# yoraish/mmd

Hardware: AMD Instinct MI355X
Metric: guided trajectories/sec (H=64, 100 denoise steps), 32-robot Empty map (higher is better)
Workload: dtype f32 (f16x2 split on the fp16 MFMA pipe: every fp32 product as 3 fp16 MFMAs, fp32 accumulate)

## Files before the change

include/mmd_amd_debug.h:

```cpp
#ifndef MMD_AMD_DEBUG_H
#define MMD_AMD_DEBUG_H

#include <stddef.h>
#include <stdint.h>

#include "mmd_amd.h"

#ifdef __cplusplus
extern "C" {
#endif

typedef struct mmd_profiler_s* mmd_profiler_t;
int mmd_profiler_create(mmd_profiler_t* out, int max_launches, int stride);
int mmd_profiler_destroy(mmd_profiler_t p);
int mmd_profiler_create_windowed(mmd_profiler_t* out, int max_launches, int stride, int window, int period);
enum { MMD_PROF_UNET = 0, MMD_PROF_STEP_GUIDED = 1, MMD_PROF_STEP_PLAIN = 2, MMD_PROF_UNET_FUSED = 3 };
int mmd_profiler_intervals(mmd_profiler_t p, int kind, double* start_ms, double* end_ms, int cap, int* n_out);
int mmd_profiler_read(mmd_profiler_t p, double* mean_ms, int* n_launches);

double mmd_unet_flops_per_trajectory(void);
double mmd_unet_mfma_flops_per_trajectory(void);
double mmd_unet_f16x2_flops_per_trajectory(void);

int mmd_sampler_stream_chunks(int n_streams, int n_robots, int samples_per_robot);

int mmd_unet_forward_profiled(mmd_unet_t unet, const float* x_dev, int t, float* eps_dev, int n_traj,
                              void* workspace_dev, size_t workspace_bytes, mmd_profiler_t profiler, void* stream);

size_t mmd_unet_weight_bytes(mmd_unet_t unet);

int mmd_unet_precision(mmd_unet_t unet);

#define MMD_TRACE_WORDS 12
int mmd_debug_ddpm_step_trace(mmd_unet_t unet, const mmd_sampler_desc* s, const mmd_guide_desc* guide, float* x_dev,
                              const float* hard_dev, int n_robots, int samples_per_robot, int i, const float* noise_dev,
                              uint64_t seed, uint32_t draw_index, void* workspace_dev, size_t workspace_bytes,
                              float* mu_dev, float* guide_chain_dev, uint32_t* trace_dev, void* stream);

#ifdef __cplusplus
}
#endif
#endif
```

mmd_amd/_lib.py:

```python
import ctypes as C
import os

_HERE = os.path.dirname(os.path.abspath(__file__))
LIB_PATH = os.path.join(_HERE, "lib", "libmmd_amd.so")
ABI_VERSION = 9
HARD_ROWS_START_GOAL = (1 << 63) | 1


def signed64(mask):
    mask = int(mask) & 0xFFFFFFFFFFFFFFFF
    return mask - (1 << 64) if mask >> 63 else mask



class ConsBins(C.Structure):
    _fields_ = [
        ("lo", C.c_float * 2), ("inv_cell", C.c_float * 2),
        ("nx", C.c_int32), ("ny", C.c_int32), ("n_all", C.c_int32), ("robot0", C.c_int32),
        ("radius", C.c_float), ("weight", C.c_float),
        ("cell_off_dev", C.c_void_p), ("entries_dev", C.c_void_p),
    ]


class GuideDesc(C.Structure):
    _fields_ = [
        ("norm_min", C.c_float * 4), ("norm_max", C.c_float * 4),
        ("limits_lo", C.c_float * 2), ("limits_hi", C.c_float * 2),
        ("grid_nx", C.c_int32), ("grid_ny", C.c_int32), ("n_grids", C.c_int32), ("n_maps", C.c_int32),
        ("sdf_grids_dev", C.c_void_p), ("robot_map_dev", C.c_void_p),
        ("ws_min", C.c_float * 2), ("ws_max", C.c_float * 2),
        ("margin", C.c_float), ("dt", C.c_float), ("sigma_gp", C.c_float),
        ("weight_collision", C.c_float), ("weight_smoothness", C.c_float), ("max_grad_norm", C.c_float),
        ("cons_ell_dev", C.c_void_p), ("grp_slot_off_dev", C.c_void_p), ("grp_weight_dev", C.c_void_p),
        ("robot_grp_off_dev", C.c_void_p), ("max_slots_per_robot", C.c_int32), ("cons_uniform_radius", C.c_float),
        ("extra_spheres_dev", C.c_void_p), ("extra_boxes_dev", C.c_void_p),
        ("n_extra_spheres", C.c_int32), ("n_extra_boxes", C.c_int32),
        ("clip_grad_rule", C.c_int32), ("max_grad_value", C.c_float),
        ("cons_bins", C.POINTER(ConsBins)),
    ]


class SamplerDesc(C.Structure):
    _fields_ = [
        ("n_diffusion_steps", C.c_int32),
        ("sqrt_recip_alphas_cumprod", C.POINTER(C.c_float)),
        ("sqrt_recipm1_alphas_cumprod", C.POINTER(C.c_float)),
        ("posterior_mean_coef1", C.POINTER(C.c_float)),
        ("posterior_mean_coef2", C.POINTER(C.c_float)),
        ("posterior_log_variance_clipped", C.POINTER(C.c_float)),
        ("n_guide_steps", C.c_int32), ("t_start_guide", C.c_int32),
        ("noise_std_extra", C.c_float), ("hard_rows", C.c_uint64), ("n_streams", C.c_int32),
        ("traj_index_base", C.c_int64), ("noise_std_extra_by_t", C.POINTER(C.c_float)), ("profiler", C.c_void_p),
        ("scale_grad_by_std", C.c_int32), ("model_predicts_x0", C.c_int32),
        ("flags", C.c_uint32), ("guide_coop_max", C.c_int32), ("robot_seeds_dev", C.c_void_p),
    ]


SAMPLER_NO_FUSED_STEP, SAMPLER_PERSIST = 1, 2
UNET_LAYERED, UNET_LAYERED_VALU = 1, 2
UNET_PRECISION_F32, UNET_PRECISION_F16 = 0, 1
UNET_PRECISIONS = {"f32": UNET_PRECISION_F32, "f16": UNET_PRECISION_F16}


class UnetOptions(C.Structure):
    _fields_ = [("flags", C.c_uint32), ("rtb_fused", C.c_int32), ("mconv_max_cs", C.c_int32), ("two_per_workgroup_max", C.c_int32),
                ("precision", C.c_int32)]


class EnsembleTile(C.Structure):
    _fields_ = [
        ("unet", C.c_void_p), ("sampler", C.POINTER(SamplerDesc)), ("guide", C.POINTER(GuideDesc)),
        ("x_dev", C.c_void_p), ("hard_dev", C.c_void_p), ("step_noise_dev", C.c_void_p), ("chain_dev", C.c_void_p),
        ("seed", C.c_uint64),
    ]


class CrossCond(C.Structure):
    _fields_ = [("m1", C.c_int32), ("m2", C.c_int32), ("ind1", C.c_int32), ("ind2", C.c_int32),
                ("rel", C.c_float * 4), ("boundary", C.c_float * 4), ("by_robot_dev", C.c_void_p)]


class AgentPath(C.Structure):
    _fields_ = [("batch_dev", C.c_void_p), ("index", C.c_int32), ("length", C.c_int32), ("start_time", C.c_int32),
                ("reserved", C.c_int32)]


class Conflict(C.Structure):
    _fields_ = [("t", C.c_int32), ("a", C.c_int32), ("b", C.c_int32), ("reserved", C.c_int32), ("pa", C.c_float * 2),
                ("pb", C.c_float * 2), ("mid", C.c_float * 2), ("reserved2", C.c_float * 2)]


class TileRef(C.Structure):
    _fields_ = [("agent", C.c_int32), ("t0", C.c_int32), ("offset", C.c_float * 2), ("rule", C.c_int32), ("reserved", C.c_int32)]


ADHERENCE_LINE, ADHERENCE_HIGHWAYS, ADHERENCE_CONVEYOR, ADHERENCE_DROP_REGION = 0, 1, 2, 3
CONFLICTS_ORDERED, CONFLICTS_PAIRS = 0, 1
SELECT_CBS, SELECT_PP = 0, 1
REPLAN_CONFLICTED, REPLAN_INDEPENDENT = 0, 1


_SIGNATURES = {
    "mmd_abi_version": (C.c_int, []),
    "mmd_last_error": (C.c_char_p, []),
    "mmd_unet_num_tensors": (C.c_int, [C.c_int, C.c_int]),
    "mmd_unet_tensor_numel": (C.c_int64, [C.c_int, C.c_int, C.c_int]),
    "mmd_unet_create": (C.c_int, [C.POINTER(C.c_void_p), C.c_int, C.c_int, C.c_int, C.POINTER(C.c_void_p),
                                  C.POINTER(C.c_int64), C.c_int, C.POINTER(UnetOptions), C.c_void_p]),
    "mmd_unet_destroy": (C.c_int, [C.c_void_p]),
    "mmd_unet_workspace_bytes": (C.c_size_t, [C.c_void_p, C.c_int]),
    "mmd_unet_forward": (C.c_int, [C.c_void_p, C.c_void_p, C.c_int, C.c_void_p, C.c_int, C.c_void_p, C.c_size_t,
                                   C.c_void_p]),
    "mmd_pack_constraints": (C.c_int, [C.c_int, C.POINTER(C.c_int32), C.POINTER(C.c_void_p), C.POINTER(C.c_void_p),
                                       C.POINTER(C.c_void_p), C.c_int, C.c_void_p, C.c_int, C.POINTER(C.c_int32)]),
    "mmd_soft_constraints_from_paths": (C.c_int, [C.c_void_p, C.c_int, C.c_int, C.c_int, C.c_int, C.c_float, C.c_float,
                                                  C.c_void_p, C.c_void_p, C.c_void_p, C.c_void_p, C.c_void_p]),
    "mmd_cons_bins_bytes": (C.c_size_t, [C.c_int, C.c_int, C.c_int, C.POINTER(C.c_size_t), C.POINTER(C.c_size_t)]),
    "mmd_bin_constraints_from_paths": (C.c_int, [C.c_void_p, C.c_int, C.c_int, C.c_float, C.POINTER(C.c_float), C.POINTER(C.c_float),
                                                 C.c_int, C.c_int, C.c_void_p, C.c_void_p, C.c_void_p]),
    "mmd_bin_paths": (C.c_int, [C.c_void_p, C.c_int, C.c_int, C.c_float, C.POINTER(C.c_float), C.POINTER(C.c_float), C.c_int, C.c_int,
                                C.c_int, C.c_void_p, C.c_void_p, C.c_void_p]),
    "mmd_guide_steps": (C.c_int, [C.POINTER(GuideDesc), C.c_void_p, C.c_void_p, C.c_uint64, C.c_int, C.c_int, C.c_int,
                                  C.c_void_p, C.c_void_p]),
    "mmd_sampler_workspace_bytes": (C.c_size_t, [C.c_void_p, C.c_int]),
    "mmd_ddpm_step": (C.c_int, [C.c_void_p, C.POINTER(SamplerDesc), C.POINTER(GuideDesc), C.c_void_p, C.c_void_p,
                                C.c_int, C.c_int, C.c_int, C.c_void_p, C.c_uint64, C.c_uint32, C.c_void_p, C.c_size_t,
                                C.c_void_p]),
    "mmd_p_sample_loop": (C.c_int, [C.c_void_p, C.POINTER(SamplerDesc), C.POINTER(GuideDesc), C.c_void_p, C.c_void_p,
                                    C.c_int, C.c_int, C.c_int, C.c_int, C.c_int, C.c_void_p, C.c_uint64, C.c_void_p,
                                    C.c_void_p, C.c_size_t, C.c_void_p]),
    "mmd_ddim_sample": (C.c_int, [C.c_void_p, C.POINTER(SamplerDesc), C.c_void_p, C.c_void_p, C.c_int, C.POINTER(GuideDesc),
                                  C.c_void_p, C.c_void_p, C.c_int, C.c_int, C.c_int, C.c_uint64, C.c_void_p, C.c_void_p,
                                  C.c_size_t, C.c_void_p]),
    "mmd_p_sample_loop_ensemble": (C.c_int, [C.POINTER(EnsembleTile), C.c_int, C.POINTER(CrossCond), C.c_int, C.c_int,
                                             C.c_int, C.c_int, C.c_int, C.c_int, C.c_void_p, C.c_size_t, C.c_void_p]),
    "mmd_q_sample": (C.c_int, [C.c_void_p, C.c_void_p, C.c_void_p, C.c_float, C.c_float, C.c_uint64, C.c_uint32,
                               C.c_int64, C.c_int, C.c_void_p]),
    "mmd_rr_collisions": (C.c_int, [C.c_void_p, C.c_int, C.c_int, C.c_float, C.c_void_p, C.c_void_p, C.c_void_p]),
    "mmd_count_collisions": (C.c_int, [C.c_void_p, C.c_void_p, C.c_int, C.c_int, C.c_int, C.c_int, C.c_int, C.c_float,
                                       C.c_void_p, C.c_void_p]),
    "mmd_count_collisions_binned": (C.c_int, [C.c_void_p, C.POINTER(ConsBins), C.c_int, C.c_int, C.c_float, C.c_void_p, C.c_void_p]),
    "mmd_path_conflicts_binned": (C.c_int, [C.c_void_p, C.POINTER(ConsBins), C.c_int, C.c_float, C.c_void_p, C.c_void_p, C.c_void_p,
                                            C.c_void_p, C.c_void_p, C.c_int, C.c_void_p]),
    "mmd_find_conflicts": (C.c_int, [C.c_void_p, C.c_int, C.c_int, C.c_float, C.c_int, C.c_void_p, C.c_void_p, C.c_void_p,
                                     C.c_void_p, C.c_int, C.c_void_p]),
    "mmd_scan_candidates": (C.c_int, [C.c_void_p, C.c_int, C.c_int, C.c_int, C.c_void_p, C.c_void_p, C.c_int, C.c_float, C.c_int,
                                      C.c_int, C.c_void_p, C.c_void_p, C.c_void_p, C.c_void_p]),
    "mmd_path_constraints": (C.c_int, [C.c_void_p, C.c_int, C.c_int, C.c_int, C.c_int, C.c_int, C.c_int, C.c_float, C.c_float,
                                       C.c_int, C.c_void_p, C.c_void_p, C.c_void_p, C.c_void_p, C.c_void_p]),
    "mmd_round_constraints_init": (C.c_int, [C.c_int, C.c_int, C.c_int, C.c_int, C.c_float, C.c_float, C.c_void_p, C.c_void_p, C.c_void_p,
                                             C.c_void_p, C.c_void_p, C.c_void_p, C.c_void_p]),
    "mmd_round_soft_from_paths": (C.c_int, [C.c_void_p, C.c_int, C.c_int, C.c_int, C.c_int, C.c_int, C.c_float, C.c_void_p, C.c_void_p]),
    "mmd_conflict_constraints_append": (C.c_int, [C.c_void_p, C.POINTER(ConsBins), C.c_int, C.c_int, C.c_int, C.c_int, C.c_float, C.c_float,
                                                  C.c_void_p, C.c_void_p, C.c_void_p, C.c_void_p]),
    "mmd_round_select": (C.c_int, [C.c_void_p, C.POINTER(ConsBins), C.c_void_p, C.c_int, C.c_int, C.c_float, C.c_int, C.c_int, C.c_void_p,
                                   C.c_void_p, C.c_void_p, C.c_void_p, C.c_void_p]),
    "mmd_framed_constraints_from_paths": (C.c_int, [C.c_void_p, C.c_void_p, C.c_int, C.c_int, C.c_int, C.c_int, C.c_int, C.c_float, C.c_float,
                                                    C.POINTER(C.c_float), C.POINTER(C.c_float), C.c_void_p, C.c_void_p, C.c_void_p, C.c_void_p,
                                                    C.c_void_p, C.c_void_p, C.c_void_p]),
    "mmd_solution_stats": (C.c_int, [C.c_void_p, C.c_int, C.c_int, C.c_float, C.c_void_p, C.c_int, C.c_void_p, C.c_void_p, C.c_void_p]),
    "mmd_postprocess_trajs": (C.c_int, [C.POINTER(GuideDesc), C.c_void_p, C.c_int, C.c_int, C.c_int, C.c_int,
                                        C.POINTER(C.c_float), C.c_float, C.POINTER(C.c_float), C.POINTER(C.c_float), C.c_int,
                                        C.c_void_p, C.c_int, C.c_void_p, C.c_void_p, C.c_void_p, C.c_void_p, C.c_void_p,
                                        C.c_void_p]),
    "mmd_select_best": (C.c_int, [C.c_void_p, C.c_void_p, C.c_void_p, C.c_void_p, C.c_int, C.c_int, C.c_void_p, C.c_void_p,
                                  C.c_void_p, C.c_void_p]),
    "mmd_points_collision": (C.c_int, [C.POINTER(GuideDesc), C.c_void_p, C.c_int, C.c_int, C.c_int, C.c_float, C.c_void_p,
                                       C.c_void_p]),
    "mmd_variance_waypoints": (C.c_int, [C.c_void_p, C.c_int, C.c_int, C.c_void_p, C.c_void_p]),
    "mmd_unnormalize_trajs": (C.c_int, [C.c_void_p, C.c_size_t, C.c_size_t, C.c_size_t, C.POINTER(C.c_float), C.POINTER(C.c_float),
                                        C.c_float, C.c_void_p, C.c_void_p, C.c_void_p]),
    "mmd_cross_condition": (C.c_int, [C.c_void_p, C.c_void_p, C.c_int, C.c_int, C.POINTER(C.c_float),
                                      C.POINTER(C.c_float), C.c_int, C.c_void_p]),
}

_DEBUG_SIGNATURES = {
    "mmd_profiler_create": (C.c_int, [C.POINTER(C.c_void_p), C.c_int, C.c_int]),
    "mmd_profiler_create_windowed": (C.c_int, [C.POINTER(C.c_void_p), C.c_int, C.c_int, C.c_int, C.c_int]),
    "mmd_profiler_intervals": (C.c_int, [C.c_void_p, C.c_int, C.POINTER(C.c_double), C.POINTER(C.c_double), C.c_int,
                                         C.POINTER(C.c_int)]),
    "mmd_profiler_destroy": (C.c_int, [C.c_void_p]),
    "mmd_profiler_read": (C.c_int, [C.c_void_p, C.POINTER(C.c_double), C.POINTER(C.c_int)]),
    "mmd_sampler_stream_chunks": (C.c_int, [C.c_int, C.c_int, C.c_int]),
    "mmd_unet_flops_per_trajectory": (C.c_double, []),
    "mmd_unet_mfma_flops_per_trajectory": (C.c_double, []),
    "mmd_unet_f16x2_flops_per_trajectory": (C.c_double, []),
    "mmd_unet_forward_profiled": (C.c_int, [C.c_void_p, C.c_void_p, C.c_int, C.c_void_p, C.c_int, C.c_void_p, C.c_size_t,
                                            C.c_void_p, C.c_void_p]),
    "mmd_unet_weight_bytes": (C.c_size_t, [C.c_void_p]),
    "mmd_unet_precision": (C.c_int, [C.c_void_p]),
    "mmd_debug_ddpm_step_trace": (C.c_int, [C.c_void_p, C.POINTER(SamplerDesc), C.POINTER(GuideDesc), C.c_void_p, C.c_void_p,
                                            C.c_int, C.c_int, C.c_int, C.c_void_p, C.c_uint64, C.c_uint32, C.c_void_p, C.c_size_t,
                                            C.c_void_p, C.c_void_p, C.c_void_p, C.c_void_p]),
}
TRACE_WORDS = 12

EXPORTED_SYMBOLS = tuple(_SIGNATURES)
DEBUG_SYMBOLS = tuple(_DEBUG_SIGNATURES)
_lib = None


def load():
    global _lib
    if _lib is None:
        if not os.path.exists(LIB_PATH):
            raise ImportError(f"{LIB_PATH} not found: the HIP extension is required (run ./build.sh or "
                              f"`python -c 'import __graft_entry__ as g; g.build()'`); there is no CPU fallback")
        lib = C.CDLL(LIB_PATH)
        for name, (res, args) in list(_SIGNATURES.items()) + list(_DEBUG_SIGNATURES.items()):
            fn = getattr(lib, name)
            fn.restype, fn.argtypes = res, args
        if lib.mmd_abi_version() != ABI_VERSION:
            raise ImportError(f"libmmd_amd.so ABI {lib.mmd_abi_version()} != expected {ABI_VERSION}")
        _lib = lib
    return _lib


def check(rc):
    if rc != 0:
        raise RuntimeError("libmmd_amd: " + load().mmd_last_error().decode())


def raw_stream(device_index=None):
    import torch
    if device_index is None:
        device_index = torch.cuda.current_device()
    get = getattr(torch._C, "_cuda_getCurrentRawStream", None)
    return int(get(device_index)) if get is not None else int(torch.cuda.current_stream(device_index).cuda_stream)


def current_stream_ptr():
    return C.c_void_p(raw_stream())


def launch(name, on, *args):
    import torch
    dev = on.device
    if dev.type != "cuda":
        raise ValueError(f"{name}: tensors must live on a CUDA(HIP) device, got {dev}")
    fn = getattr(_lib if _lib is not None else load(), name)
    cur = torch.cuda.current_device()
    if dev.index is None or dev.index == cur:
        rc = fn(*args, C.c_void_p(raw_stream(cur)))
    else:
        with torch.cuda.device(dev):
            rc = fn(*args, C.c_void_p(raw_stream(dev.index)))
    if rc != 0:
        check(rc)


def require_gpu(t, name="tensor"):
    import torch
    if not (isinstance(t, torch.Tensor) and t.is_cuda and t.dtype == torch.float32 and t.is_contiguous()):
        raise ValueError(f"{name} must be a contiguous float32 CUDA(HIP) tensor")
    return C.c_void_p(t.data_ptr())
```

mmd_amd/csrc/f16x2.h:

```cpp
#pragma once
#include <hip/hip_runtime.h>

#include <cmath>
#include <cstdint>
#include <cstring>
#include <vector>

namespace mmd {

typedef float f32x4 __attribute__((ext_vector_type(4)));

struct DynScale { float s, inv; };
__device__ __forceinline__ DynScale dyn_scale(float M) {
  unsigned eb = (__float_as_uint(M) >> 23) & 0xffu;
  eb = eb < 64u ? 64u : eb;
  return DynScale{__uint_as_float((264u - eb) << 23), __uint_as_float((eb - 10u) << 23)};
}
typedef _Float16 f16x8 __attribute__((ext_vector_type(8)));
typedef _Float16 f16x2 __attribute__((ext_vector_type(2)));
typedef float f32x2 __attribute__((ext_vector_type(2)));
typedef unsigned u32x4 __attribute__((ext_vector_type(4)));

struct F16Pair { unsigned hi, lo; };
__device__ __forceinline__ F16Pair f16_split2(float v0, float v1) {
  const f16x2 h = __builtin_convertvector(f32x2{v0, v1}, f16x2);
  const unsigned hb = __builtin_bit_cast(unsigned, h);
  float d0, d1;
  asm("v_fma_mix_f32 %0, %1, -1.0, %2 op_sel_hi:[1,0,0]" : "=v"(d0) : "v"(hb), "v"(v0));
  asm("v_fma_mix_f32 %0, %1, -1.0, %2 op_sel:[1,0,0] op_sel_hi:[1,0,0]" : "=v"(d1) : "v"(hb), "v"(v1));
  const f16x2 l = __builtin_convertvector(f32x2{d0, d1}, f16x2);
  return F16Pair{hb, __builtin_bit_cast(unsigned, l)};
}
__device__ __forceinline__ f32x4 mfma_h(const u32x4& a, const u32x4& b, const f32x4& c) {
  return __builtin_amdgcn_mfma_f32_16x16x32_f16(__builtin_bit_cast(f16x8, a), __builtin_bit_cast(f16x8, b), c, 0, 0, 0);
}
template <bool ZERO>
__device__ __forceinline__ void vb_three(f32x4& x, const u32x4 (&a)[2], const u32x4 (&b)[2]) {
  const f32x4 z = {0.f, 0.f, 0.f, 0.f};
  f32x4 c = ZERO ? z : x;
  c = mfma_h(a[1], b[0], c);
  c = mfma_h(a[0], b[1], c);
  c = mfma_h(a[0], b[0], c);
  x = c;
#ifndef MMD_VB3_LOOSE
  __builtin_amdgcn_sched_barrier(0);
#endif
}

static inline float f16_scale_for(float m) {
  if (!(m > 0.f) || !std::isfinite(m)) return 1.f;
  int ex;
  (void)frexpf(m, &ex);
  return ldexpf(1.f, 15 - ex);
}
static inline void f16_split_host(float u, float scale, uint16_t (&piece)[2]) {
  const float us = u * scale;
  const _Float16 h = (_Float16)us;
  const _Float16 l = (_Float16)(us - (float)h);
  memcpy(&piece[0], &h, 2);
  memcpy(&piece[1], &l, 2);
}
static size_t push_inverse(std::vector<float>& blob, const std::vector<float>& sc, float in_scale = 1.f) {
  while (blob.size() % 4) blob.push_back(0.f);
  const size_t off = blob.size();
  for (float v : sc) blob.push_back(1.f / (v * in_scale));
  while (blob.size() % 4) blob.push_back(0.f);
  return off;
}

static inline float rd_w(const float* w, int cout, int cin_full, int ks, bool transposed, int n, int ci, int k) {
  return transposed ? w[((size_t)ci * cout + n) * ks + k] : w[((size_t)n * cin_full + ci) * ks + k];
}
static std::vector<float> rd_col_scales(const float* w, int cout, int cin_full, int ks, const std::vector<int>& kidx, bool transposed) {
  std::vector<float> sc(cout);
  for (int n = 0; n < cout; ++n) {
    float m = 0.f;
    for (int ci = 0; ci < cin_full; ++ci)
      for (int k : kidx) m = fmaxf(m, fabsf(rd_w(w, cout, cin_full, ks, transposed, n, ci, k)));
    sc[n] = f16_scale_for(m);
  }
  return sc;
}
static size_t pack_rd(std::vector<float>& blob, const float* w, int cout, int cin_full, int c_lo, int cin_chunk, int ks,
                      const std::vector<int>& kidx, bool transposed, bool pair_cols, const std::vector<float>& sc) {
  while (blob.size() % 4) blob.push_back(0.f);
  const size_t base = blob.size();
  const int tiles = cout / 16, KC = cin_chunk / 32, T = (int)kidx.size();
  const size_t frags = (size_t)tiles * T * KC * 2;
  blob.resize(base + (frags + 8) * 64 * 4, 0.f);
  uint16_t* out = reinterpret_cast<uint16_t*>(blob.data() + base);
  for (int t = 0; t < tiles; ++t)
    for (int tap = 0; tap < T; ++tap)
      for (int kc = 0; kc < KC; ++kc)
        for (int lane = 0; lane < 64; ++lane)
          for (int j = 0; j < 8; ++j) {
            const int n = pair_cols ? (t / 2) * 32 + 2 * (lane & 15) + (t & 1) : 16 * t + (lane & 15);
            const int ci = c_lo + 8 * (KC * (lane >> 4) + kc) + j;
            uint16_t piece[2];
            f16_split_host(rd_w(w, cout, cin_full, ks, transposed, n, ci, kidx[tap]), sc[n], piece);
            for (int q = 0; q < 2; ++q) out[(((((size_t)t * T + tap) * KC + kc) * 2 + q) * 64 + lane) * 8 + j] = piece[q];
          }
  return base;
}

}
```

mmd_amd/csrc/unet.hip:

```cpp
#include <hip/hip_runtime.h>

#include <cmath>
#include <cstring>
#include <memory>
#include <vector>

#include "../../include/mmd_amd.h"
#include "../../include/mmd_amd_debug.h"
#include "common.h"
#include "f16x2.h"
#include "guide_dev.h"
#include "unet_kernel.h"
#include "unet_spec.h"

namespace mmd {

__device__ __forceinline__ float mish_exact(float y) {
  float sp = y > 20.f ? y : log1pf(expf(y));
  return y * tanhf(sp);
}

__global__ void time_table_kernel(TimeArgs a) {
  __shared__ float emb[32], h1[128], m[32];
  const int t = blockIdx.x, tid = threadIdx.x;
  if (tid < 16) {
    const float f = expf((float)tid * -(logf(10000.f) / 15.f));
    const float v = (float)t * f;
    emb[tid] = sinf(v);
    emb[tid + 16] = cosf(v);
  }
  __syncthreads();
  {
    float s = a.b1[tid];
    for (int k = 0; k < 32; ++k) s += a.w1[tid * 32 + k] * emb[k];
    h1[tid] = mish_exact(s);
  }
  __syncthreads();
  if (tid < 32) {
    float s = a.b3[tid];
    for (int k = 0; k < 128; ++k) s += a.w3[tid * 128 + k] * h1[k];
    m[tid] = mish_exact(s);
  }
  __syncthreads();
  for (int r = 0; r < a.n_rtb; ++r)
    for (int c = tid; c < a.cout[r]; c += 128) {
      float s = a.cb[r][c];
      for (int k = 0; k < 32; ++k) s += a.cw[r][c * 32 + k] * m[k];
      a.table[(size_t)t * a.total + a.off[r] + c] = s;
    }
}


static inline bool fused_config(int uid, int n_levels) { return uid == 32 && n_levels == 3; }

void launch_time_table(const TimeArgs& a, int T, hipStream_t st) { hipLaunchKernelGGL(time_table_kernel, dim3(T), dim3(128), 0, st, a); }

static size_t pack_im2col4(std::vector<float>& blob, const float* w, int cout, bool is_res, const std::vector<float>& sc) {
  while (blob.size() % 4) blob.push_back(0.f);
  const size_t base = blob.size();
  const int tiles = cout / 16;
  blob.resize(base + ((size_t)tiles * 2 + 8) * 64 * 4, 0.f);
  uint16_t* out = reinterpret_cast<uint16_t*>(blob.data() + base);
  for (int t = 0; t < tiles; ++t)
    for (int lane = 0; lane < 64; ++lane)
      for (int jj = 0; jj < 8; ++jj) {
        const int n = (t / 2) * 32 + 2 * (lane & 15) + (t & 1), tap = 2 * (lane >> 4) + (jj >> 2), c = jj & 3;
        float v = 0.f;
        if (is_res) v = tap == 2 ? w[(size_t)n * 4 + c] : 0.f;
        else if (tap < 5) v = w[((size_t)n * 4 + c) * 5 + tap];
        uint16_t piece[2];
        f16_split_host(v, sc[n], piece);
        for (int q = 0; q < 2; ++q) out[(((size_t)t * 2 + q) * 64 + lane) * 8 + jj] = piece[q];
      }
  return base;
}
static size_t pack_rd_res(std::vector<float>& blob, const float* wres, int cout, int cin_full, int c_lo, int cin_chunk,
                          bool pair_cols, const std::vector<float>& sc) {
  return pack_rd(blob, wres, cout, cin_full, c_lo, cin_chunk, 1, std::vector<int>{0}, false, pair_cols, sc);
}

static std::vector<std::vector<float>> time_bias_absmax(const float* const* tensors, const Spec& s, int T) {
  auto mish = [](double y) { return y * std::tanh(y > 20.0 ? y : std::log1p(std::exp(y))); };
  const float *w1 = tensors[s.t_time[0]], *b1 = tensors[s.t_time[1]], *w3 = tensors[s.t_time[2]], *b3 = tensors[s.t_time[3]];
  std::vector<std::vector<float>> mxv(s.rtb.size());
  for (size_t r = 0; r < s.rtb.size(); ++r) mxv[r].assign(s.rtb[r].cout, 0.f);
  for (int t = 0; t < T; ++t) {
    double emb[32], h1[128], m[32];
    for (int i = 0; i < 16; ++i) {
      const double f = std::exp((double)i * -(std::log(10000.0) / 15.0)), v = (double)t * f;
      emb[i] = std::sin(v); emb[i + 16] = std::cos(v);
    }
    for (int j = 0; j < 128; ++j) { double a = b1[j]; for (int k = 0; k < 32; ++k) a += (double)w1[j * 32 + k] * emb[k]; h1[j] = mish(a); }
    for (int j = 0; j < 32; ++j) { double a = b3[j]; for (int k = 0; k < 128; ++k) a += (double)w3[j * 128 + k] * h1[k]; m[j] = mish(a); }
    for (size_t r = 0; r < s.rtb.size(); ++r) {
      const float *cw = tensors[s.rtb[r].t_cw], *cb = tensors[s.rtb[r].t_cb];
      for (int c = 0; c < s.rtb[r].cout; ++c) {
        double a = cb[c];
        for (int k = 0; k < 32; ++k) a += (double)cw[c * 32 + k] * m[k];
        mxv[r][c] = fmaxf(mxv[r][c], (float)std::fabs(a));
      }
    }
  }
  return mxv;
}
static float static_act_scale(const float* gamma, const float* beta, const std::vector<float>& tbmax, int c) {
  float B = 0.f;
  for (int i = 0; i < c; ++i) B = fmaxf(B, fmaxf(0.31f, 16.f * fabsf(gamma[i]) + fabsf(beta[i])) + tbmax[i] * 1.001f);
  if (!std::isfinite(B)) return 1.f;
  int ex;
  (void)frexpf(B, &ex);
  return ldexpf(1.f, 10 - (ex - 1));
}


struct ConvW { size_t bias, gamma, beta, wbf, isc; };
struct RtbW { ConvW a, b; size_t res_bias, res_isc, res_bf, res_c1_bf; int tb_off; size_t a_c1_bf; float act_a; };
struct TailW { size_t bias, wbf[2], isc[2]; };

struct UnetPack {
  int tb_total = 0;
  RtbW rtb[12];
  TailW down[2], up[2];
  ConvW fin;
  size_t fin_w1 = 0, fin_b1 = 0, fin_is1 = 0;
  float fin_act = 1.f;
  size_t raw_time[4], raw_cw[12], raw_cb[12];
};

}

using namespace mmd;

struct mmd_unet_s {
  mmd::LayeredUnet* layered = nullptr;
  int T = 0;
  int precision = MMD_UNET_PRECISION_F32;
  int ns2_max = 512;
#ifndef MMD_NS1_MAX
#define MMD_NS1_MAX 256
#endif
  int ns1_max = MMD_NS1_MAX;
  size_t blob_bytes = 0;
  float* blob = nullptr;
  float* ttable = nullptr;
  mmd::UnetPack w;
};

namespace mmd {

static size_t push(std::vector<float>& blob, const float* p, int64_t n) {
  while (blob.size() % 4) blob.push_back(0.f);
  size_t off = blob.size();
  blob.insert(blob.end(), p, p + n);
  while (blob.size() % 4) blob.push_back(0.f);
  return off;
}

enum ConvAForm { A_IM2COL4, A_FIRST_WHOLE, A_FIRST_CAT, A_IDENT };
struct BlockPack { const char* name; bool pairs; ConvAForm a; };
static const BlockPack kBlockPack[12] = {
    {"d00", true, A_IM2COL4},    {"d01", true, A_IDENT},  {"d10", true, A_FIRST_WHOLE}, {"d11", true, A_IDENT},
    {"d20", true, A_FIRST_WHOLE}, {"d21", true, A_IDENT}, {"u00", false, A_FIRST_CAT},  {"u01", false, A_IDENT},
    {"u10", true, A_FIRST_CAT},  {"u11", true, A_IDENT},  {"mid1", true, A_IDENT},      {"mid2", true, A_IDENT}};

static void pack_unet(const Spec& s, const float* const* tensors, int T, std::vector<float>& blob, UnetPack& p) {
  const std::vector<int> taps5 = {0, 1, 2, 3, 4}, taps3 = {0, 1, 2}, taps1 = {0};
  for (int i = 0; i < 4; ++i) p.raw_time[i] = push(blob, tensors[s.t_time[i]], s.numel[s.t_time[i]]);
  int tb_off = 0;
  const std::vector<std::vector<float>> tbmax = time_bias_absmax(tensors, s, T);
  for (int r = 0; r < 12; ++r) {
    const Rtb& R = s.rtb[r];
    const BlockPack& B = kBlockPack[r];
    RtbW& W = p.rtb[r];
    W = RtbW{};
    while (blob.size() % 4) blob.push_back(0.f);
    {
      const std::vector<float> sc = rd_col_scales(tensors[R.t_w0], R.cout, R.cin, 5, taps5, false);
      W.a.isc = push_inverse(blob, sc);
      if (B.a == A_IDENT) {
        W.a.wbf = pack_rd(blob, tensors[R.t_w0], R.cout, R.cin, 0, R.cin, 5, taps5, false, B.pairs, sc);
      } else {
        const float* wres = tensors[R.t_rw];
        const std::vector<float> scr = rd_col_scales(wres, R.cout, R.cin, 1, taps1, false);
        W.res_isc = push_inverse(blob, scr);
        if (B.a == A_IM2COL4) {
          W.a.wbf = pack_im2col4(blob, tensors[R.t_w0], R.cout, false, sc);
          W.res_bf = pack_im2col4(blob, wres, R.cout, true, scr);
        } else {
          const int chunk = B.a == A_FIRST_WHOLE ? R.cin : R.cin / 2;
          W.a.wbf = pack_rd(blob, tensors[R.t_w0], R.cout, R.cin, 0, chunk, 5, taps5, false, B.pairs, sc);
          W.res_bf = pack_rd_res(blob, wres, R.cout, R.cin, 0, chunk, B.pairs, scr);
          if (B.a == A_FIRST_CAT) {
            W.a_c1_bf = pack_rd(blob, tensors[R.t_w0], R.cout, R.cin, chunk, chunk, 5, taps5, false, B.pairs, sc);
            W.res_c1_bf = pack_rd_res(blob, wres, R.cout, R.cin, chunk, chunk, B.pairs, scr);
          }
        }
      }
    }
    W.a.bias = push(blob, tensors[R.t_b0], R.cout);
    W.a.gamma = push(blob, tensors[R.t_g0], R.cout);
    W.a.beta = push(blob, tensors[R.t_be0], R.cout);
    {
      W.act_a = static_act_scale(tensors[R.t_g0], tensors[R.t_be0], tbmax[r], R.cout);
      const std::vector<float> sc = rd_col_scales(tensors[R.t_w1], R.cout, R.cout, 5, taps5, false);
      W.b.isc = push_inverse(blob, sc, W.act_a);
      W.b.wbf = pack_rd(blob, tensors[R.t_w1], R.cout, R.cout, 0, R.cout, 5, taps5, false, B.pairs, sc);
    }
    W.b.bias = push(blob, tensors[R.t_b1], R.cout);
    W.b.gamma = push(blob, tensors[R.t_g1], R.cout);
    W.b.beta = push(blob, tensors[R.t_be1], R.cout);
    p.raw_cw[r] = push(blob, tensors[R.t_cw], (int64_t)R.cout * 32);
    p.raw_cb[r] = push(blob, tensors[R.t_cb], R.cout);
    W.res_bias = R.res ? push(blob, tensors[R.t_rb], R.cout) : 0;
    W.tb_off = tb_off;
    tb_off += R.cout;
  }
  p.tb_total = tb_off;
  for (int i = 0; i < 2; ++i) {
    const int c = s.dims[i + 1];
    p.down[i].bias = push(blob, tensors[s.t_down[i][1]], c);
    {
      const std::vector<float> sct = rd_col_scales(tensors[s.t_down[i][0]], c, c, 3, taps3, false);
      p.down[i].isc[0] = push_inverse(blob, sct);
      p.down[i].wbf[0] = pack_rd(blob, tensors[s.t_down[i][0]], c, c, 0, c, 3, taps3, false, true, sct);
    }
    const int cu = s.dims[2 - i];
    p.up[i].bias = push(blob, tensors[s.t_up[i][1]], cu);
    {
      const std::vector<int> ke = {3, 1}, ko = {2, 0};
      const std::vector<float> sce = rd_col_scales(tensors[s.t_up[i][0]], cu, cu, 4, ke, true);
      const std::vector<float> sco = rd_col_scales(tensors[s.t_up[i][0]], cu, cu, 4, ko, true);
      p.up[i].isc[0] = push_inverse(blob, sce);
      p.up[i].isc[1] = push_inverse(blob, sco);
      p.up[i].wbf[0] = pack_rd(blob, tensors[s.t_up[i][0]], cu, cu, 0, cu, 4, ke, true, i == 1, sce);
      p.up[i].wbf[1] = pack_rd(blob, tensors[s.t_up[i][0]], cu, cu, 0, cu, 4, ko, true, i == 1, sco);
    }
  }
  {
    const std::vector<float> sc = rd_col_scales(tensors[s.t_final[0]], 32, 32, 5, taps5, false);
    p.fin.isc = push_inverse(blob, sc);
    p.fin.wbf = pack_rd(blob, tensors[s.t_final[0]], 32, 32, 0, 32, 5, taps5, false, true, sc);
    p.fin.bias = push(blob, tensors[s.t_final[1]], 32);
    p.fin.gamma = push(blob, tensors[s.t_final[2]], 32);
    p.fin.beta = push(blob, tensors[s.t_final[3]], 32);
    p.fin_act = static_act_scale(tensors[s.t_final[2]], tensors[s.t_final[3]], std::vector<float>(32, 0.f), 32);
    std::vector<float> sc1 = rd_col_scales(tensors[s.t_final[4]], 4, 32, 1, taps1, false);
    p.fin_is1 = push_inverse(blob, sc1, p.fin_act);
    std::vector<float> w1(16 * 32, 0.f);
    memcpy(w1.data(), tensors[s.t_final[4]], sizeof(float) * 4 * 32);
    sc1.resize(16, 1.f);
    p.fin_w1 = pack_rd(blob, w1.data(), 16, 32, 0, 32, 1, taps1, false, false, sc1);
    p.fin_b1 = push(blob, tensors[s.t_final[5]], 4);
  }
}

static int fill_time_table(const mmd_unet_s* u, const Spec& s, hipStream_t st) {
  const UnetPack& p = u->w;
  TimeArgs ta{};
  ta.w1 = u->blob + p.raw_time[0]; ta.b1 = u->blob + p.raw_time[1];
  ta.w3 = u->blob + p.raw_time[2]; ta.b3 = u->blob + p.raw_time[3];
  for (int r = 0; r < 12; ++r) {
    ta.cw[r] = u->blob + p.raw_cw[r]; ta.cb[r] = u->blob + p.raw_cb[r];
    ta.cout[r] = s.rtb[r].cout; ta.off[r] = p.rtb[r].tb_off;
  }
  ta.n_rtb = 12; ta.total = p.tb_total; ta.table = u->ttable;
  launch_time_table(ta, u->T, st);
  MMD_HIP_CHECK(hipGetLastError());
  MMD_HIP_CHECK(hipStreamSynchronize(st));
  return 0;
}

static RtbPtrs rtb_ptrs(const mmd_unet_s* u, const RtbW& w, int t) {
  RtbPtrs p{};
  p.ba = u->blob + w.a.bias; p.ga = u->blob + w.a.gamma; p.bea = u->blob + w.a.beta;
  p.tb = u->ttable + (size_t)t * u->w.tb_total + w.tb_off;
  p.bb = u->blob + w.b.bias; p.gb = u->blob + w.b.gamma; p.beb = u->blob + w.b.beta;
  p.wa_bf = w.a.wbf ? reinterpret_cast<const uint4*>(u->blob + w.a.wbf) : nullptr;
  p.wb_bf = w.b.wbf ? reinterpret_cast<const uint4*>(u->blob + w.b.wbf) : nullptr;
  p.isa = w.a.wbf ? u->blob + w.a.isc : nullptr;
  p.isb = w.b.wbf ? u->blob + w.b.isc : nullptr;
  p.act_a = w.act_a;
  return p;
}

static ChainArgs args_chain(const mmd_unet_s* u, const int* rtb, int n_ident, const TailW* tail, const float* in0, int t, int n) {
  ChainArgs a{};
  a.in0 = in0; a.n = n;
  const RtbW& w0 = u->w.rtb[rtb[0]];
  a.r0 = rtb_ptrs(u, w0, t);
  a.wa0_c1_bf = w0.a_c1_bf ? reinterpret_cast<const uint4*>(u->blob + w0.a_c1_bf) : nullptr;
  a.br = u->blob + w0.res_bias;
  a.isr = w0.res_isc ? u->blob + w0.res_isc : nullptr;
  a.wres_bf = w0.res_bf ? reinterpret_cast<const uint4*>(u->blob + w0.res_bf) : nullptr;
  a.wres_c1_bf = w0.res_c1_bf ? reinterpret_cast<const uint4*>(u->blob + w0.res_c1_bf) : nullptr;
  for (int k = 0; k < n_ident; ++k) a.ri[k] = rtb_ptrs(u, u->w.rtb[rtb[1 + k]], t);
  if (tail) {
    a.bt = u->blob + tail->bias;
    a.wt_bf0 = reinterpret_cast<const uint4*>(u->blob + tail->wbf[0]);
    a.ist0 = u->blob + tail->isc[0];
    if (tail->wbf[1]) {
      a.wt_bf1 = reinterpret_cast<const uint4*>(u->blob + tail->wbf[1]);
      a.ist1 = u->blob + tail->isc[1];
    }
  }
  return a;
}

static UnetArgs unet_args(const mmd_unet_s* u, const float* x, int t, int n, float* eps) {
  static const int kD0[] = {0, 1}, kD1[] = {2, 3}, kD2[] = {4, 5, 10, 11}, kU0[] = {6, 7}, kU1[] = {8, 9};
  const UnetPack& p = u->w;
  UnetArgs a{};
  a.n = n;
  a.c[0] = args_chain(u, kD0, 1, &p.down[0], x, t, n);
  a.c[1] = args_chain(u, kD1, 1, &p.down[1], nullptr, t, n);
  a.c[2] = args_chain(u, kD2, 3, nullptr, nullptr, t, n);
  a.c[3] = args_chain(u, kU0, 1, &p.up[0], nullptr, t, n);
  a.c[4] = args_chain(u, kU1, 1, &p.up[1], nullptr, t, n);
  a.fin.out = eps;
  a.fin.w5 = reinterpret_cast<const uint4*>(u->blob + p.fin.wbf);
  a.fin.isc = u->blob + p.fin.isc;
  a.fin.bias = u->blob + p.fin.bias; a.fin.gamma = u->blob + p.fin.gamma; a.fin.beta = u->blob + p.fin.beta;
  a.fin.act = p.fin_act;
  a.fin.w1_bf = reinterpret_cast<const uint4*>(u->blob + p.fin_w1);
  a.fin.is1 = u->blob + p.fin_is1;
  a.fin.w1_bias = u->blob + p.fin_b1;
  return a;
}

int unet_forward_fused(mmd_unet_t u, const float* x, int t, float* eps, int n, void* ws, size_t ws_bytes, Profiler* prof,
                       hipStream_t st, const FusedStep& fs) {
  MMD_REQUIRE(u && x && eps && ws, "mmd_unet_forward: NULL argument");
  MMD_REQUIRE(n >= 1, "mmd_unet_forward: n_traj must be >= 1");
  MMD_REQUIRE(t >= 0 && t < u->T, "mmd_unet_forward: t=%d outside [0,%d)", t, u->T);
  MMD_REQUIRE(ws_bytes >= mmd_unet_workspace_bytes(u, n), "mmd_unet_forward: workspace too small");
  if (u->layered) {
    MMD_REQUIRE(!fs.enabled, "mmd_unet_forward: the fused unguided step exists in the fused kernel only");
    const bool bracket = prof_begin(prof, 0, MMD_PROF_UNET, st);
    const int rc = layered_forward(u->layered, x, t, eps, n, ws, ws_bytes, st);
    if (bracket) prof_end(prof, st);
    return rc;
  }
  UnetArgs a = unet_args(u, x, t, n, eps);
  a.fs = fs;
  const bool bracket = prof_begin(prof, 0, fs.enabled ? MMD_PROF_UNET_FUSED : MMD_PROF_UNET, st);
  int rc = 0;
  if (u->precision == MMD_UNET_PRECISION_F16) {
    const int ns = n <= u->ns1_max && n <= u->ns2_max ? 1 : n <= u->ns2_max ? 2 : 4;
    rc = launch_unet_f16(ns, (n + ns - 1) / ns, st, &a, sizeof(a));
  } else if (n <= u->ns1_max && n <= u->ns2_max) hipLaunchKernelGGL(unet_kernel<1>, dim3(n), dim3(256), 0, st, a);
  else if (n <= u->ns2_max) hipLaunchKernelGGL(unet_kernel<2>, dim3((n + 1) / 2), dim3(256), 0, st, a);
  else hipLaunchKernelGGL(unet_kernel<4>, dim3((n + 3) / 4), dim3(256), 0, st, a);
  if (bracket) prof_end(prof, st);
  if (rc) return rc;
  MMD_HIP_CHECK(hipGetLastError());
  return 0;
}

int unet_persist_steps(mmd_unet_t u, int n, void* ws, size_t ws_bytes, hipStream_t st, const FusedStep* steps, int n_steps) {
  MMD_REQUIRE(u && !u->layered && ws && n >= 1, "unet_persist_steps: bad arguments");
  MMD_REQUIRE(n_steps >= 1 && n_steps <= PERSIST_MAX_STEPS && ws_bytes >= (size_t)PERSIST_TABLE_BYTES, "unet_persist_steps: step table");
  for (int s = 0; s < n_steps; ++s) MMD_REQUIRE(steps[s].t_row >= 0 && steps[s].t_row < u->T, "unet_persist_steps: t outside the time table");
  MMD_HIP_CHECK(hipMemcpyAsync(ws, steps, sizeof(FusedStep) * n_steps, hipMemcpyHostToDevice, st));
  char* const args_dev = reinterpret_cast<char*>(ws) + PERSIST_ARGS_OFF;
  const UnetArgs a = unet_args(u, reinterpret_cast<const float*>(steps[0].x), 0, n, nullptr);
  MMD_HIP_CHECK(hipMemcpyAsync(args_dev, &a, sizeof(a), hipMemcpyHostToDevice, st));
  const FusedStep* sd = reinterpret_cast<const FusedStep*>(ws);
  const UnetArgs* ap = reinterpret_cast<const UnetArgs*>(args_dev);
  if (u->precision == MMD_UNET_PRECISION_F16) {
    const int ns = n <= u->ns2_max ? 2 : 4;
    if (int rc = launch_unet_persist_f16(ns, (n + ns - 1) / ns, st, args_dev, sizeof(a), sd, n_steps, u->w.tb_total)) return rc;
  } else if (n <= u->ns2_max) hipLaunchKernelGGL(unet_persist_kernel<2>, dim3((n + 1) / 2), dim3(256), 0, st, ap, sd, n_steps, u->w.tb_total);
  else hipLaunchKernelGGL(unet_persist_kernel<4>, dim3((n + 3) / 4), dim3(256), 0, st, ap, sd, n_steps, u->w.tb_total);
  MMD_HIP_CHECK(hipGetLastError());
  return 0;
}
bool unet_fused_step_supported(mmd_unet_t u) { return u && !u->layered; }

static constexpr double rtb_flops(double cin, double cout, double L) {
  return 2.0 * cout * 5 * cin * L + 2.0 * cout * 5 * cout * L + (cin != cout ? 2.0 * cout * cin * L : 0.0);
}
static const double kUnetFlops =
    rtb_flops(4, 32, 64) + rtb_flops(32, 32, 64) + 2.0 * 32 * 3 * 32 * 32 +
    rtb_flops(32, 64, 32) + rtb_flops(64, 64, 32) + 2.0 * 64 * 3 * 64 * 16 +
    rtb_flops(64, 128, 16) + 3 * rtb_flops(128, 128, 16) +
    rtb_flops(256, 64, 16) + rtb_flops(64, 64, 16) + 2.0 * 64 * 4 * 64 * 16 +
    rtb_flops(128, 32, 32) + rtb_flops(32, 32, 32) + 2.0 * 32 * 4 * 32 * 32 +
    2.0 * 32 * 5 * 32 * 64 + 2.0 * 4 * 32 * 64;

static constexpr double d5(double cin, double cout, double L) { return 2.0 * cout * 5 * cin * L; }
static const double kF16Flops =
    2 * (2.0 * 32 * 32 * 64) + 3 * d5(32, 32, 64) + 2.0 * 32 * 3 * 32 * 32 +
    d5(32, 64, 32) + 2.0 * 64 * 32 * 32 + 3 * d5(64, 64, 32) + 2.0 * 64 * 3 * 64 * 16 +
    d5(64, 128, 16) + 2.0 * 128 * 64 * 16 + 7 * d5(128, 128, 16) +
    d5(256, 64, 16) + 2.0 * 64 * 256 * 16 + 3 * d5(64, 64, 16) + 2.0 * 64 * 4 * 64 * 16 +
    d5(128, 32, 32) + 2.0 * 32 * 128 * 32 + 3 * d5(32, 32, 32) + 2.0 * 32 * 4 * 32 * 32 +
    d5(32, 32, 64) + 2.0 * 16 * 32 * 64;
static const double kFp32Flops = 0.0;
static const double kUnetMfmaFlops = kF16Flops + kFp32Flops;
}

extern "C" {

int mmd_unet_num_tensors(int unet_input_dim, int n_levels) {
  Spec s;
  if (!build_spec(unet_input_dim, n_levels, s)) {
    set_error("unsupported TemporalUnet configuration (unet_input_dim=%d, n_levels=%d)", unet_input_dim, n_levels);
    return -1;
  }
  return (int)s.numel.size();
}

int64_t mmd_unet_tensor_numel(int unet_input_dim, int n_levels, int index) {
  Spec s;
  if (!build_spec(unet_input_dim, n_levels, s) || index < 0 || index >= (int)s.numel.size()) return -1;
  return s.numel[index];
}

int mmd_unet_create(mmd_unet_t* out, int unet_input_dim, int n_levels, int n_diffusion_steps,
                    const float* const* tensors, const int64_t* numels, int n_tensors, const mmd_unet_options* options,
                    void* stream) {
  Spec s;
  MMD_REQUIRE(out != nullptr, "mmd_unet_create: out is NULL");
  MMD_REQUIRE(build_spec(unet_input_dim, n_levels, s),
              "unsupported TemporalUnet configuration (unet_input_dim=%d, n_levels=%d)", unet_input_dim, n_levels);
  MMD_REQUIRE(n_tensors == (int)s.numel.size(), "expected %d parameter tensors, got %d", (int)s.numel.size(), n_tensors);
  for (int i = 0; i < n_tensors; ++i)
    MMD_REQUIRE(numels[i] == s.numel[i] && tensors[i] != nullptr, "parameter tensor %d has %lld elements, expected %lld",
                i, (long long)numels[i], (long long)s.numel[i]);
  MMD_REQUIRE(n_diffusion_steps >= 1, "n_diffusion_steps must be >= 1");
  const int precision = options ? options->precision : MMD_UNET_PRECISION_F32;
  const bool layered_path = !fused_config(unet_input_dim, n_levels) || (options && (options->flags & MMD_UNET_LAYERED));
  MMD_REQUIRE(precision == MMD_UNET_PRECISION_F32 || precision == MMD_UNET_PRECISION_F16,
              "mmd_unet_options.precision = %d: MMD_UNET_PRECISION_F32 (0) or MMD_UNET_PRECISION_F16 (1)", precision);
  MMD_REQUIRE(precision == MMD_UNET_PRECISION_F32 || !layered_path,
              "mmd_unet_options.precision = MMD_UNET_PRECISION_F16 exists in the fused kernel only (unet_input_dim 32, 3 levels, "
              "without MMD_UNET_LAYERED): unet_input_dim=%d, n_levels=%d, flags=%u", unet_input_dim, n_levels, options->flags);
  hipStream_t st = (hipStream_t)stream;

  struct Destroy { void operator()(mmd_unet_s* p) const { (void)mmd_unet_destroy(p); } };
  std::unique_ptr<mmd_unet_s, Destroy> u(new mmd_unet_s());
  u->T = n_diffusion_steps;
  u->precision = precision;
  if (options && options->two_per_workgroup_max != 0) u->ns2_max = options->two_per_workgroup_max < 0 ? 0 : options->two_per_workgroup_max;
  if (layered_path) {
    if (int rc = layered_create(&u->layered, s, n_diffusion_steps, tensors, options, st)) return rc;
  } else {
    std::vector<float> blob;
    pack_unet(s, tensors, n_diffusion_steps, blob, u->w);
    if (hipMalloc(&u->blob, blob.size() * sizeof(float)) != hipSuccess ||
        hipMalloc(&u->ttable, (size_t)u->T * u->w.tb_total * sizeof(float)) != hipSuccess) {
      set_error("mmd_unet_create: hipMalloc failed");
      return 1;
    }
    MMD_HIP_CHECK(hipMemcpyAsync(u->blob, blob.data(), blob.size() * sizeof(float), hipMemcpyHostToDevice, st));
    MMD_HIP_CHECK(hipStreamSynchronize(st));
    u->blob_bytes = blob.size() * sizeof(float);
    if (int rc = fill_time_table(u.get(), s, st)) return rc;
  }
  *out = u.release();
  return 0;
}

int mmd_unet_destroy(mmd_unet_t u) {
  if (!u) return 0;
  layered_destroy(u->layered);
  if (u->blob) (void)hipFree(u->blob);
  if (u->ttable) (void)hipFree(u->ttable);
  delete u;
  return 0;
}

size_t mmd_unet_workspace_bytes(mmd_unet_t u, int n_traj) {
  if (u && u->layered) return layered_workspace_bytes(u->layered, n_traj);
  return n_traj > 0 ? PERSIST_TABLE_BYTES : 0;
}

int mmd_unet_forward(mmd_unet_t u, const float* x, int t, float* eps, int n, void* ws, size_t ws_bytes, void* stream) {
  return unet_forward_fused(u, x, t, eps, n, ws, ws_bytes, nullptr, (hipStream_t)stream, FusedStep{});
}

#ifdef MMD_TRACE
int mmd_debug_set_trace(void* dev_ptr) {
  return hipMemcpyToSymbol(HIP_SYMBOL(g_trace), &dev_ptr, sizeof(dev_ptr)) == hipSuccess ? 0 : 1;
}
#endif

int mmd_unet_precision(mmd_unet_t u) { return u ? u->precision : -1; }

size_t mmd_unet_weight_bytes(mmd_unet_t u) {
  if (!u) return 0;
  return u->layered ? layered_weight_bytes(u->layered) : u->blob_bytes;
}

double mmd_unet_flops_per_trajectory(void) { return kUnetFlops; }
double mmd_unet_mfma_flops_per_trajectory(void) { return kUnetMfmaFlops; }
double mmd_unet_f16x2_flops_per_trajectory(void) { return kF16Flops; }

}
```

mmd_amd/csrc/unet_kernel.h:

```cpp
#pragma once
#include <hip/hip_runtime.h>

#include <cmath>
#include <cstdlib>
#include <cstring>
#include <type_traits>
#include <vector>

#include "../../include/mmd_amd.h"
#include "../../include/mmd_amd_debug.h"
#include "common.h"
#include "f16x2.h"
#include "gn_mish.h"
#include "guide_dev.h"
#include "unet_spec.h"

#ifdef MMD_UNET_F16
#define MMD_LO(...)
namespace mmd {
namespace f16 {
constexpr int N_PIECES = 1;
struct F16Pair { unsigned hi; };
__device__ __forceinline__ F16Pair f16_split2(float v0, float v1) {
  return F16Pair{__builtin_bit_cast(unsigned, __builtin_convertvector(f32x2{v0, v1}, f16x2))};
}
template <bool ZERO>
__device__ __forceinline__ void vb_three(f32x4& x, const u32x4 (&a)[2], const u32x4 (&b)[2]) {
  const f32x4 z = {0.f, 0.f, 0.f, 0.f};
  x = mfma_h(a[0], b[0], ZERO ? z : x);
  __builtin_amdgcn_sched_barrier(0);
}
#else
#define MMD_LO(...) __VA_ARGS__
namespace mmd {
constexpr int N_PIECES = 2;
#endif

struct FinalArgs {
  float* out;
  const uint4* w5;
  const float* isc;
  const float* bias;
  const float* gamma;
  const float* beta;
  float act;
  const uint4* w1_bf;
  const float* is1;
  const float* w1_bias;
};

template <int NT> struct Epi { float b[NT], g[NT], be[NT], is[NT], tb[NT]; };
template <int NT>
__device__ __forceinline__ Epi<NT> epi_load(const float* b, const float* g, const float* be, const float* tb, const float* isc, int c0) {
  Epi<NT> e;
#pragma unroll
  for (int t = 0; t < NT; ++t) {
    e.b[t] = b[c0 + t];
    e.g[t] = g[c0 + t];
    e.be[t] = be[c0 + t];
    e.is[t] = isc ? isc[c0 + t] : 1.f;
    e.tb[t] = tb ? tb[c0 + t] : 0.f;
  }
  return e;
}

struct RowPair { float a, b; };
__device__ __forceinline__ RowPair rows_xor16(float v) {
  const unsigned u = __builtin_bit_cast(unsigned, v);
  const auto r = __builtin_amdgcn_permlane16_swap(u, u, false, false);
  return RowPair{__builtin_bit_cast(float, (unsigned)r[0]), __builtin_bit_cast(float, (unsigned)r[1])};
}
__device__ __forceinline__ RowPair rows_xor32(float v) {
  const unsigned u = __builtin_bit_cast(unsigned, v);
  const auto r = __builtin_amdgcn_permlane32_swap(u, u, false, false);
  return RowPair{__builtin_bit_cast(float, (unsigned)r[0]), __builtin_bit_cast(float, (unsigned)r[1])};
}
__device__ __forceinline__ float add_xor16(float v) { const RowPair r = rows_xor16(v); return r.a + r.b; }
__device__ __forceinline__ float add_xor32(float v) { const RowPair r = rows_xor32(v); return r.a + r.b; }
__device__ __forceinline__ float max_nn(float a, float b) {
  const unsigned ua = __builtin_bit_cast(unsigned, a), ub = __builtin_bit_cast(unsigned, b);
  return __builtin_bit_cast(float, __builtin_elementwise_max(ua, ub));
}
__device__ __forceinline__ float max_xor16(float v) { const RowPair r = rows_xor16(v); return max_nn(r.a, r.b); }
__device__ __forceinline__ float max_xor32(float v) { const RowPair r = rows_xor32(v); return max_nn(r.a, r.b); }

template <int CTRL>
__device__ __forceinline__ float dpp_max(float v) {
  return max_nn(v, __builtin_bit_cast(float, __builtin_amdgcn_update_dpp(0, __builtin_bit_cast(int, v), CTRL, 0xF, 0xF, true)));
}
__device__ __forceinline__ float row_max16(float v) {
  v = dpp_max<0xB1>(v);
  v = dpp_max<0x4E>(v);
  v = dpp_max<0x141>(v);
  v = dpp_max<0x140>(v);
  return v;
}
__device__ __forceinline__ float wave_max(float v) {
  v = row_max16(v);
  v = max_xor16(v);
  return max_xor32(v);
}
constexpr int MX_SLOTS = 8;
constexpr int MX_REGION = 4 * MX_SLOTS;
constexpr int MX_FLOATS = 3 * MX_REGION;

#ifdef MMD_NO_PIN
#define MMD_PIN_LOADS() do { } while (0)
#else
#define MMD_PIN_LOADS()                 \
  do {                                  \
    asm volatile("" ::: "memory");      \
    __builtin_amdgcn_sched_barrier(0);  \
  } while (0)
#endif

#ifdef MMD_TRACE
__device__ unsigned long long* g_trace = nullptr;
#define TR(tag)                                                                                                       \
  do {                                                                                                                \
    if (g_trace && (threadIdx.x & 63) == 0)                                                                           \
      g_trace[((size_t)blockIdx.x * 4 + (threadIdx.x >> 6)) * 256 + (tag)] = wall_clock64();                          \
  } while (0)
#else
#define TR(tag) do { } while (0)
#endif

__device__ __forceinline__ int opaque_tid() {
  int tid = threadIdx.x;
  asm volatile("" : "+v"(tid));
  return tid;
}
template <int CTRL>
__device__ __forceinline__ float dpp_add(float v) {
  return v + __builtin_bit_cast(float, __builtin_amdgcn_update_dpp(0, __builtin_bit_cast(int, v), CTRL, 0xF, 0xF, true));
}
constexpr int MAX_IDENT = 3;

struct RtbPtrs {
  const float* ba; const float* ga; const float* bea; const float* tb;
  const float* bb; const float* gb; const float* beb;
  const uint4* wa_bf; const uint4* wb_bf;
  const float* isa; const float* isb;
  float act_a;
};

struct ChainArgs {
  const float* in0;
  RtbPtrs r0;
  const uint4* wa0_c1_bf;
  const float* br;
  const float* isr;
  const uint4* wres_bf;
  const uint4* wres_c1_bf;
  const uint4* wt_bf0; const uint4* wt_bf1;
  const float* ist0; const float* ist1;
  RtbPtrs ri[MAX_IDENT];
  const float* bt;
  int n;
};

struct D2 {
  static constexpr int N_IDENT = 3, MID_AFTER = 1, C0 = 64, XSTR = C0 + 2, SROWS = 16 + 4;
  static constexpr int XSS = SROWS * XSTR + (16 - (SROWS * XSTR) % 32 + 32) % 32;
  static constexpr int SLAB_OFF = (4 * XSS * 4 + 255) / 256 * 256;
  static_assert(N_IDENT <= MAX_IDENT && MID_AFTER >= 1, "ChainArgs::ri holds the identity RTBs");
};

constexpr int cmax(int a, int b) { return a > b ? a : b; }
constexpr int MX_OFF = (D2::SLAB_OFF + 43008) / 4 + 8;
constexpr int PARK2_OFF = MX_OFF + MX_FLOATS;
constexpr int UNET_LDS_FLOATS = PARK2_OFF + 3 * 256 * 4;
static_assert(UNET_LDS_FLOATS * 4 == 76960, "LDS of a workgroup");

template <int NT>
__device__ __forceinline__ Epi<NT> epi_a(const RtbPtrs& R, int tb_off, int c0) { return epi_load<NT>(R.ba, R.ga, R.bea, R.tb + tb_off, R.isa, c0); }
template <int NT>
__device__ __forceinline__ Epi<NT> epi_b(const RtbPtrs& R, int c0) { return epi_load<NT>(R.bb, R.gb, R.beb, nullptr, R.isb, c0); }

typedef const __attribute__((address_space(1))) char* WBase;
__device__ __forceinline__ WBase wave_uniform_base(const void* p, unsigned byte_off) {
  const unsigned long long a = reinterpret_cast<unsigned long long>(p) + byte_off;
  const unsigned lo = __builtin_amdgcn_readfirstlane((unsigned)a), hi = __builtin_amdgcn_readfirstlane((unsigned)(a >> 32));
  return (WBase)(((unsigned long long)hi << 32) | lo);
}
template <int NT> struct WTiles {
  WBase base[NT];
  unsigned off;
  __device__ __forceinline__ u32x4 frag(int t, int i) const {
    const int adv = (i + 4) / 8 * 8192;
    unsigned long long b = reinterpret_cast<unsigned long long>(base[t]) + adv;
    if (adv) asm("" : "+s"(b));
    return *reinterpret_cast<const __attribute__((address_space(1))) u32x4*>((WBase)b + (i * 1024 - adv) + off);
  }
};
template <int NT>
__device__ __forceinline__ WTiles<NT> w_tiles(const void* w, int frags, int tile0, int lane) {
  WTiles<NT> r;
#pragma unroll
  for (int t = 0; t < NT; ++t) r.base[t] = wave_uniform_base(w, (unsigned)(tile0 + t) * (unsigned)frags * 1024u);
  r.off = (unsigned)lane * 16u;
  return r;
}
template <int NT> struct WStaged {
  const u32x4* p[NT];
  __device__ __forceinline__ u32x4 frag(int t, int i) const { return p[t][i * 64]; }
};
template <int NT>
__device__ __forceinline__ WStaged<NT> w_staged(const char* wb, int frags, int lane) {
  WStaged<NT> r;
#pragma unroll
  for (int t = 0; t < NT; ++t) r.p[t] = reinterpret_cast<const u32x4*>(wb) + t * frags * 64 + lane;
  return r;
}
template <int NT> __device__ __forceinline__ u32x4 w_frag(const WTiles<NT>& w, int t, int i) { return w.frag(t, i); }
template <int NT> __device__ __forceinline__ u32x4 w_frag(const WStaged<NT>& w, int t, int i) { return w.frag(t, i); }
__device__ __forceinline__ u32x4 w_frag(const u32x4* const* w, int t, int i) { return w[t][i * 64]; }
template <int NT> __device__ __forceinline__ WTiles<NT> w_local(WTiles<NT> w) {
  asm volatile("" : "+v"(w.off));
  return w;
}
template <int NT> __device__ __forceinline__ WStaged<NT> w_local(const WStaged<NT>& w) { return w; }
__device__ __forceinline__ const u32x4* const* w_local(const u32x4* const* w) { return w; }
template <int NT> __device__ __forceinline__ WTiles<NT> w_local(WTiles<NT> w, const WTiles<NT>& first) {
  w.off = first.off;
  return w;
}
template <class W, class F> __device__ __forceinline__ auto w_local(const W& w, const F&) { return w_local(w); }

constexpr bool ring_prefetch(int m_tiles) {
#ifdef MMD_NO_PF
  return false;
#else
  return m_tiles <= 2;
#endif
}

template <int M, int N>
__device__ __forceinline__ void tile_scale(f32x4 (&t)[M][N], float s) {
#pragma unroll
  for (int m = 0; m < M; ++m)
#pragma unroll
    for (int n = 0; n < N; ++n) t[m][n] *= s;
}
template <int M, int N>
__device__ __forceinline__ void tile_copy(f32x4 (&d)[M][N], const f32x4 (&s)[M][N]) {
#pragma unroll
  for (int m = 0; m < M; ++m)
#pragma unroll
    for (int n = 0; n < N; ++n) d[m][n] = s[m][n];
}
template <int M, int N, int S>
__device__ __forceinline__ void tile_finish_res(f32x4 (&r)[M][N], const float (&isr)[N], const float (&inv)[S], const float (&br)[N]) {
#pragma unroll
  for (int m = 0; m < M; ++m)
#pragma unroll
    for (int n = 0; n < N; ++n) r[m][n] = r[m][n] * (isr[n] * inv[m / (M / S)]) + br[n];
}
template <int M, int N>
__device__ __forceinline__ void tile_finish_res(f32x4 (&r)[M][N], const float (&isr)[N], float inv, const float (&br)[N]) {
  const float inv1[1] = {inv};
  tile_finish_res(r, isr, inv1, br);
}
template <int MS, int M, int N>
__device__ __forceinline__ f32x4 (&sub_tile(f32x4 (&t)[M][N], int m0))[MS][N] { return reinterpret_cast<f32x4(&)[MS][N]>(t[m0]); }
template <int MS, int M, int N>
__device__ __forceinline__ const f32x4 (&sub_tile(const f32x4 (&t)[M][N], int m0))[MS][N] { return reinterpret_cast<const f32x4(&)[MS][N]>(t[m0]); }

template <int NT> struct AddTimeBias {
  static constexpr bool ACT = true;
  float tb[NT];
  ActScale as;
  __device__ __forceinline__ float operator()(int, int t, int) const { return tb[t]; }
};
template <int MT, int NT> struct AddResidual {
  static constexpr bool ACT = false;
  const f32x4 (&res)[MT][NT];
  ActScale as;
  __device__ __forceinline__ float operator()(int mt, int t, int r) const { return res[mt][t][r]; }
};
template <int NT>
__device__ __forceinline__ AddTimeBias<NT> gn_addend(const Epi<NT>& e, float act_s) {
  AddTimeBias<NT> a;
#pragma unroll
  for (int t = 0; t < NT; ++t) a.tb[t] = e.tb[t] * act_s;
  a.as = act_scale(act_s);
  return a;
}
template <int MT, int NT>
__device__ __forceinline__ AddResidual<MT, NT> gn_addend(const Epi<NT>&, const f32x4 (&res)[MT][NT]) { return AddResidual<MT, NT>{res, ActScale{}}; }

template <int CPG>
__device__ __forceinline__ float group_colsum(float v) {
  v = dpp_add<0xB1>(v);
  v = dpp_add<0x4E>(v);
  if constexpr (CPG >= 8) v = dpp_add<0x141>(v);
  if constexpr (CPG >= 16) v = dpp_add<0x140>(v);
  return v;
}


template <int C> struct RdGeo {
  static constexpr int KC = C / 32, RPS = 20, BX = 4 * RPS * 16 + 32, G = (KC * BX + 255) / 256 * 256, PS = 4 * G, BYTES = 2 * PS;
  static constexpr int FRAGS5 = 5 * KC * 2;
  static constexpr int tile_row(int m) { return m * RPS; }
};
template <int C> struct RlGeo {
  static constexpr int KC = C / 32, RPS = 36, BX = 4 * RPS * 16 + 32, G = (KC * BX + 255) / 256 * 256, PS = 4 * G, BYTES = 2 * PS;
  static constexpr int FRAGS5 = 5 * KC * 2, FRAGS3 = 3 * KC * 2;
  static constexpr int tile_row(int m) { return (m >> 1) * RPS + (m & 1) * 16; }
};
template <class GEO>
__device__ __forceinline__ void rd_zero_halo(char* slab) {
  constexpr int TOT = N_PIECES * 4 * GEO::KC * 4 * 4;
  for (int idx = opaque_tid(); idx < TOT; idx += 256) {
    const int hr = idx & 3, sm = (idx >> 2) & 3, blk = (idx >> 4) % (4 * GEO::KC), q = idx / (64 * GEO::KC);
    *reinterpret_cast<uint4*>(slab + q * GEO::PS + (blk / GEO::KC) * GEO::G + (blk % GEO::KC) * GEO::BX +
                              (sm * GEO::RPS + (hr < 2 ? hr : GEO::RPS - 4 + hr)) * 16) = make_uint4(0u, 0u, 0u, 0u);
  }
}
template <class GEO, int NT, class W>
__device__ __forceinline__ void rd_load_b(u32x4 (&b)[NT][2], const W& w, int step) {
#pragma unroll
  for (int t = 0; t < NT; ++t)
#pragma unroll
    for (int q = 0; q < 2; ++q) b[t][q] = w_frag(w, t, step * 2 + q);
}
template <class GEO, int SM = 2>
__device__ __forceinline__ void rd_load_a(u32x4 (&a)[SM][2], const char* va, int rowoff, int kc, int hp) {
#pragma unroll
  for (int sm = 0; sm < SM; ++sm)
#pragma unroll
    for (int q = 0; q < 2; ++q)
      a[sm][q] = *reinterpret_cast<const u32x4*>(va + q * GEO::PS + kc * GEO::BX + (GEO::tile_row(SM * hp + sm) + rowoff) * 16);
}
constexpr int RD_RD = 2;
#ifndef MMD_D2_RD
#define MMD_D2_RD 3
#endif
#ifndef MMD_D1_RD
#define MMD_D1_RD 3
#endif
#ifndef MMD_U0C_RD
#define MMD_U0C_RD 4
#endif
#ifndef MMD_U0_RD
#define MMD_U0_RD 3
#endif
template <class GEO, int NT, int RD = RD_RD, class W>
__device__ __forceinline__ void rd_ring_load(u32x4 (&b)[RD][NT][2], const W& w_in) {
  const auto w = w_local(w_in);
#pragma unroll
  for (int i = 0; i < RD; ++i) rd_load_b<GEO, NT>(b[i], w, i);
  MMD_PIN_LOADS();
}
template <class GEO, int NT, int TAP0, int TAPS, bool FRESH, bool RES, int MT = 4, int RD = RD_RD, class W, class WR>
__device__ __forceinline__ void rd_taps(f32x4 (&acc)[MT][NT], f32x4 (&res)[MT][NT], const char* va, const W& w_in, const WR& wr_in,
                                        u32x4 (&b)[RD][NT][2]) {
  const auto w = w_local(w_in);
  [[maybe_unused]] const auto wr = w_local(wr_in, w);
  constexpr int KC = GEO::KC, STEPS = TAPS * KC, SM = MT >= 2 ? 2 : 1, HP = MT / SM;
  static_assert(MT == 1 || MT % 2 == 0, "M tiles are processed in pairs");
  u32x4 a[2][SM][2];
  rd_load_a<GEO, SM>(a[0], va, TAP0, 0, 0);
  constexpr int C0 = (2 - TAP0) * KC;
  constexpr int RES_LOOK = C0 < 3 ? C0 : 3;
  u32x4 brp[RES ? KC : 1][NT][2];
  auto load_br = [&](int kc) {
#pragma unroll
    for (int t = 0; t < NT; ++t)
#pragma unroll
      for (int q = 0; q < 2; ++q) brp[kc][t][q] = w_frag(wr, t, kc * 2 + q);
  };
#pragma unroll
  for (int tap = 0; tap < TAPS; ++tap)
#pragma unroll
    for (int kc = 0; kc < KC; ++kc) {
      const int st = tap * KC + kc, ri = st % RD;
      const bool zero = FRESH && st == 0, last_kc = kc + 1 == KC, with_res = RES && TAP0 + tap == 2;
      if constexpr (RES) {
        if (st + RES_LOOK >= C0 && st + RES_LOOK < C0 + KC) load_br(st + RES_LOOK - C0);
      }
#pragma unroll
      for (int hp = 0; hp < HP; ++hp) {
        const int cur = (st * HP + hp) & 1;
        if (hp + 1 < HP) rd_load_a<GEO, SM>(a[cur ^ 1], va, TAP0 + tap, kc, hp + 1);
        else rd_load_a<GEO, SM>(a[cur ^ 1], va, last_kc ? TAP0 + tap + 1 : TAP0 + tap, last_kc ? 0 : kc + 1, 0);
        MMD_PIN_LOADS();
        const u32x4(&ac)[SM][2] = a[cur];
        const u32x4(&bc)[NT][2] = b[ri];
#pragma unroll
        for (int sm = 0; sm < SM; ++sm)
#pragma unroll
          for (int t = 0; t < NT; ++t) {
            if (zero) vb_three<true>(acc[SM * hp + sm][t], ac[sm], bc[t]);
            else vb_three<false>(acc[SM * hp + sm][t], ac[sm], bc[t]);
          }
        if constexpr (RES) {
          if (with_res) {
#pragma unroll
            for (int sm = 0; sm < SM; ++sm)
#pragma unroll
              for (int t = 0; t < NT; ++t) {
                const u32x4(&bw)[2] = brp[kc][t];
                if (FRESH && kc == 0) vb_three<true>(res[SM * hp + sm][t], ac[sm], bw);
                else vb_three<false>(res[SM * hp + sm][t], ac[sm], bw);
              }
          }
        }
      }
      if (st + RD < STEPS) rd_load_b<GEO, NT>(b[ri], w, st + RD);
      MMD_PIN_LOADS();
    }
}
template <int NT, int NG, bool ACT, class ADD, int NS>
__device__ __forceinline__ void rd_gn_mish(f32x4 (&acc)[NS][NT], const float (&bias)[NT], const float (&gamma)[NT],
                                           const float (&beta)[NT], const float (&isc)[NT], const float (&inv)[NS],
                                           const ActScale& as, ADD add) {
  constexpr float inv_n = 1.f / (float)NG;
  float bsum = 0.f;
#pragma unroll
  for (int t = 0; t < NT; ++t) bsum += bias[t];
  const float bmean = group_colsum<8>(bsum) * 16.f * inv_n;
  float k[NS][NT], sum[NS], dm[NS][NT], sq[NS];
#pragma unroll
  for (int sm = 0; sm < NS; ++sm) {
    float v = 0.f;
#pragma unroll
    for (int t = 0; t < NT; ++t) {
      k[sm][t] = isc[t] * inv[sm];
      v = fmaf((acc[sm][t][0] + acc[sm][t][1]) + (acc[sm][t][2] + acc[sm][t][3]), k[sm][t], v);
    }
    sum[sm] = group_colsum<8>(v);
  }
#pragma unroll
  for (int sm = 0; sm < NS; ++sm) sum[sm] = add_xor16(sum[sm]);
#pragma unroll
  for (int sm = 0; sm < NS; ++sm) sum[sm] = add_xor32(sum[sm]);
#pragma unroll
  for (int sm = 0; sm < NS; ++sm) {
    const float mean = fmaf(sum[sm], inv_n, bmean);
    float v = 0.f;
#pragma unroll
    for (int t = 0; t < NT; ++t) {
      dm[sm][t] = mean - bias[t];
#pragma unroll
      for (int r = 0; r < 4; ++r) {
        const float d = fmaf(acc[sm][t][r], k[sm][t], -dm[sm][t]);
        v = fmaf(d, d, v);
      }
    }
    sq[sm] = group_colsum<8>(v);
  }
#pragma unroll
  for (int sm = 0; sm < NS; ++sm) sq[sm] = add_xor16(sq[sm]);
#pragma unroll
  for (int sm = 0; sm < NS; ++sm) sq[sm] = add_xor32(sq[sm]);
#pragma unroll
  for (int sm = 0; sm < NS; ++sm) {
    const float rstd = __builtin_amdgcn_rsqf(fmaf(sq[sm], inv_n, 1e-5f));
#pragma unroll
    for (int t = 0; t < NT; ++t) {
      GnCoef cf = gn_coef(dm[sm][t], rstd, gamma[t], beta[t]);
      cf.sa *= k[sm][t];
#pragma unroll
      for (int r = 0; r < 4; r += 2) {
        const f32x2_t o = gn_mish2<ACT>(f32x2_t{acc[sm][t][r], acc[sm][t][r + 1]}, cf, f32x2_t{add(sm, t, r), add(sm, t, r + 1)}, as);
        acc[sm][t][r] = o.x;
        acc[sm][t][r + 1] = o.y;
      }
    }
  }
}
template <int NG, int NS, int NT, class ADDEND>
__device__ __forceinline__ void rd_gn(f32x4 (&acc)[NS][NT], const Epi<NT>& e, const float (&inv)[NS], const ADDEND& addend) {
  const auto add = gn_addend(e, addend);
  rd_gn_mish<NT, NG, decltype(add)::ACT>(acc, e.b, e.g, e.be, e.is, inv, add.as, add);
}
template <int NT, int NS>
__device__ __forceinline__ void rd_dyn_out(const f32x4 (&acc)[NS][NT], float* mx, int wave, int lane, int region2) {
#pragma unroll
  for (int sm = 0; sm < NS; ++sm) {
    float m = 0.f;
#pragma unroll
    for (int t = 0; t < NT; ++t)
#pragma unroll
      for (int r = 0; r < 4; ++r) m = fmaxf(m, fabsf(acc[sm][t][r]));
    m = row_max16(m);
    m = max_xor16(m);
    if ((lane & 31) == 0) {
      mx[sm * MX_SLOTS + 2 * wave + (lane >> 5)] = m;
      if (region2) mx[region2 * MX_REGION + sm * MX_SLOTS + 2 * wave + (lane >> 5)] = m;
    }
  }
}
__device__ __forceinline__ float mx_read(const float* mx, int sm) {
  const float4 p = *reinterpret_cast<const float4*>(mx + sm * MX_SLOTS), q = *reinterpret_cast<const float4*>(mx + sm * MX_SLOTS + 4);
  return max_nn(max_nn(max_nn(p.x, p.y), max_nn(p.z, p.w)), max_nn(max_nn(q.x, q.y), max_nn(q.z, q.w)));
}
template <int M, int N, int S>
__device__ __forceinline__ void mx_scale_tile(const float* mx, int s0, f32x4 (&t)[M][N], float (&inv)[S]) {
#pragma unroll
  for (int sl = 0; sl < S; ++sl) {
    const DynScale ds = dyn_scale(mx_read(mx, s0 + sl));
    inv[sl] = ds.inv;
    tile_scale(sub_tile<M / S>(t, M / S * sl), ds.s);
  }
}
template <class GEO, int NS>
__device__ __forceinline__ void rd_store2(char* vs, const f32x4 (&acc)[NS][2]) {
#pragma unroll
  for (int sm = 0; sm < NS; ++sm)
#pragma unroll
    for (int r = 0; r < 4; ++r) {
      const F16Pair f = f16_split2(acc[sm][0][r], acc[sm][1][r]);
      *reinterpret_cast<unsigned*>(vs + (sm * GEO::RPS + r) * 16) = f.hi;
      MMD_LO(*reinterpret_cast<unsigned*>(vs + GEO::PS + (sm * GEO::RPS + r) * 16) = f.lo;)
    }
}
template <class GEO, int NS>
__device__ __forceinline__ void rd_store1(char* vs, const f32x4 (&acc)[NS][1], int lane) {
  constexpr int HS = NS / 2;
  const bool odd = lane & 1;
  if constexpr (NS == 1) {
#pragma unroll
    for (int r = 0; r < 4; ++r) {
      const float own = acc[0][0][r];
      const float recv = __builtin_bit_cast(float, __builtin_amdgcn_update_dpp(0, __builtin_bit_cast(int, own), 0xB1, 0xf, 0xf, true));
      const F16Pair f = f16_split2(odd ? recv : own, odd ? own : recv);
      *reinterpret_cast<unsigned*>(vs + r * 16) = f.hi;
      MMD_LO(*reinterpret_cast<unsigned*>(vs + GEO::PS + r * 16) = f.lo;)
    }
  }
#pragma unroll
  for (int h = 0; h < HS; ++h)
#pragma unroll
    for (int r = 0; r < 4; ++r) {
      const float send = odd ? acc[h][0][r] : acc[HS + h][0][r];
      const float recv = __builtin_bit_cast(float, __builtin_amdgcn_update_dpp(0, __builtin_bit_cast(int, send), 0xB1, 0xf, 0xf, true));
      const float own = odd ? acc[HS + h][0][r] : acc[h][0][r];
      const F16Pair f = f16_split2(odd ? recv : own, odd ? own : recv);
      char* p = vs + ((odd ? HS + h : h) * GEO::RPS + r) * 16;
      *reinterpret_cast<unsigned*>(p) = f.hi;
      MMD_LO(*reinterpret_cast<unsigned*>(p + GEO::PS) = f.lo;)
    }
}
template <int C, int XSS, int XSTR, int NS>
__device__ __forceinline__ void rowform_to_rd(const float* xslab, char* slab, const float* mx) {
  using GEO = RdGeo<C>;
  constexpr int CP2 = C / 2, ITEMS = 16 * NS * CP2;
  static_assert(ITEMS % 256 == 0 && XSTR % 2 == 0, "items per thread; 8-byte aligned channel pairs");
  const int tid = opaque_tid();
#pragma unroll
  for (int it = 0; it < ITEMS / 256; ++it) {
    const int idx = it * 256 + tid;
    const int cp = idx % CP2, sp = idx / CP2, sm = sp >> 4, pos = sp & 15;
    const float sc = dyn_scale(mx_read(mx, sm)).s;
    const float2 t = *reinterpret_cast<const float2*>(xslab + sm * XSS + (2 + pos) * XSTR + 2 * cp);
    const F16Pair f = f16_split2(t.x * sc, t.y * sc);
    const int blk = cp >> 2;
    char* dst = slab + (blk / GEO::KC) * GEO::G + (blk % GEO::KC) * GEO::BX + (sm * GEO::RPS + 2 + pos) * 16 + (cp & 3) * 4;
    *reinterpret_cast<unsigned*>(dst) = f.hi;
    MMD_LO(*reinterpret_cast<unsigned*>(dst + GEO::PS) = f.lo;)
  }
}

template <int C, int L> struct RwGeo {
  static constexpr int KC = C / 32, RPS = 16, ROWS = L + 4, BX = ROWS * 16 + 32, G = (KC * BX + 255) / 256 * 256, PS = 4 * G;
  static constexpr int BYTES = 2 * PS, FRAGS5 = 5 * KC * 2, FRAGS3 = 3 * KC * 2;
  static constexpr int tile_row(int m) { return m * RPS; }
};
template <class GEO, int SROWS, int TILES_PER_SAMPLE> struct Stride2 : GEO {
  static constexpr int tile_row(int m) { return (m / TILES_PER_SAMPLE) * SROWS + (m % TILES_PER_SAMPLE) * 32; }
};
__device__ __forceinline__ float wave_sum_rows(float v) {
  v = add_xor16(v);
  v = add_xor32(v);
  return v;
}
template <int GL>
__device__ __forceinline__ float rw_gsum(float v) {
  v = dpp_add<0xB1>(v);
  if constexpr (GL >= 4) v = dpp_add<0x4E>(v);
  if constexpr (GL >= 8) v = dpp_add<0x141>(v);
  return wave_sum_rows(v);
}
template <int MT, int NT, int GL, int NG, bool ACT, class ADD>
__device__ __forceinline__ void rw_gn_mish(f32x4 (&acc)[MT][NT], const float (&bias)[NT], const float (&gamma)[NT],
                                           const float (&beta)[NT], const float (&isc)[NT], float inv, const ActScale& as, ADD add) {
  constexpr float inv_n = 1.f / (float)NG;
  float k[NT], bsum = 0.f, v = 0.f;
#pragma unroll
  for (int t = 0; t < NT; ++t) {
    k[t] = isc[t] * inv;
    bsum += bias[t];
    float st = 0.f;
#pragma unroll
    for (int mt = 0; mt < MT; ++mt) st += (acc[mt][t][0] + acc[mt][t][1]) + (acc[mt][t][2] + acc[mt][t][3]);
    v = fmaf(st, k[t], v);
  }
  const float mean = (rw_gsum<GL>(v) + rw_gsum<GL>(bsum) * (float)(4 * MT)) * inv_n;
  float dm[NT], q = 0.f;
#pragma unroll
  for (int t = 0; t < NT; ++t) {
    dm[t] = mean - bias[t];
#pragma unroll
    for (int mt = 0; mt < MT; ++mt)
#pragma unroll
      for (int r = 0; r < 4; ++r) {
        const float d = fmaf(acc[mt][t][r], k[t], -dm[t]);
        q = fmaf(d, d, q);
      }
  }
  const float rstd = __builtin_amdgcn_rsqf(fmaf(rw_gsum<GL>(q), inv_n, 1e-5f));
#pragma unroll
  for (int t = 0; t < NT; ++t) {
    GnCoef cf = gn_coef(dm[t], rstd, gamma[t], beta[t]);
    cf.sa *= k[t];
#pragma unroll
    for (int mt = 0; mt < MT; ++mt)
#pragma unroll
      for (int r = 0; r < 4; r += 2) {
        const f32x2_t o = gn_mish2<ACT>(f32x2_t{acc[mt][t][r], acc[mt][t][r + 1]}, cf, f32x2_t{add(mt, t, r), add(mt, t, r + 1)}, as);
        acc[mt][t][r] = o.x;
        acc[mt][t][r + 1] = o.y;
      }
  }
}
struct HalfStat { float mean, m2; };
template <int HT, int NT, int GL, int NG>
__device__ __forceinline__ HalfStat rw_half_stat(const f32x4 (&acc)[HT][NT], const float (&bias)[NT], const float (&k)[NT], float bsum4) {
  float v = 0.f;
#pragma unroll
  for (int t = 0; t < NT; ++t) {
    float st = (acc[0][t][0] + acc[0][t][1]) + (acc[0][t][2] + acc[0][t][3]);
    if constexpr (HT == 2) st += (acc[1][t][0] + acc[1][t][1]) + (acc[1][t][2] + acc[1][t][3]);
    v = fmaf(st, k[t], v);
  }
  HalfStat h;
  h.mean = (rw_gsum<GL>(v) + bsum4 * (float)(4 * HT)) * (2.f / (float)NG);
  float q = 0.f;
#pragma unroll
  for (int t = 0; t < NT; ++t) {
    const float dm = h.mean - bias[t];
#pragma unroll
    for (int mt = 0; mt < HT; ++mt)
#pragma unroll
      for (int r = 0; r < 4; ++r) {
        const float d = fmaf(acc[mt][t][r], k[t], -dm);
        q = fmaf(d, d, q);
      }
  }
  h.m2 = rw_gsum<GL>(q);
  return h;
}
struct GnStat { float mean, rstd; };
template <int NG>
__device__ __forceinline__ GnStat gn_combine(const HalfStat& h0, const HalfStat& h1) {
  const float dlt = h1.mean - h0.mean;
  const float m2 = fmaf(dlt * dlt, 0.25f * (float)NG, h0.m2 + h1.m2);
  return GnStat{0.5f * (h0.mean + h1.mean), __builtin_amdgcn_rsqf(fmaf(m2, 1.f / (float)NG, 1e-5f))};
}
template <int MT, int NT, bool ACT, class ADD>
__device__ __forceinline__ void rw_gn_apply(f32x4 (&acc)[MT][NT], const float (&bias)[NT], const float (&gamma)[NT],
                                            const float (&beta)[NT], const float (&k)[NT], const GnStat& st, const ActScale& as, ADD add) {
#pragma unroll
  for (int t = 0; t < NT; ++t) {
    GnCoef cf = gn_coef(st.mean - bias[t], st.rstd, gamma[t], beta[t]);
    cf.sa *= k[t];
#pragma unroll
    for (int mt = 0; mt < MT; ++mt)
#pragma unroll
      for (int r = 0; r < 4; r += 2) {
        const f32x2_t o = gn_mish2<ACT>(f32x2_t{acc[mt][t][r], acc[mt][t][r + 1]}, cf, f32x2_t{add(mt, t, r), add(mt, t, r + 1)}, as);
        acc[mt][t][r] = o.x;
        acc[mt][t][r + 1] = o.y;
      }
  }
}
template <int GL, int NT>
__device__ __forceinline__ float rw_gn_prologue(const float (&bias)[NT], const float (&isc)[NT], float inv, float (&k)[NT]) {
  float bsum = 0.f;
#pragma unroll
  for (int t = 0; t < NT; ++t) {
    k[t] = isc[t] * inv;
    bsum += bias[t];
  }
  return rw_gsum<GL>(bsum);
}
template <int MT, int NT, int GL, int NG, bool ACT, class ADD>
__device__ __forceinline__ void rw_gn_mish_whole(f32x4 (&acc)[MT][NT], const float (&bias)[NT], const float (&gamma)[NT],
                                                 const float (&beta)[NT], const float (&isc)[NT], float inv, const ActScale& as, ADD add) {
  constexpr int HT = MT / 2;
  static_assert(MT == 2 || MT == 4, "two halves of one or two M tiles");
  float k[NT];
  const float bsum4 = rw_gn_prologue<GL>(bias, isc, inv, k);
  const HalfStat h0 = rw_half_stat<HT, NT, GL, NG>(sub_tile<HT>(acc, 0), bias, k, bsum4);
  const HalfStat h1 = rw_half_stat<HT, NT, GL, NG>(sub_tile<HT>(acc, HT), bias, k, bsum4);
  rw_gn_apply<MT, NT, ACT>(acc, bias, gamma, beta, k, gn_combine<NG>(h0, h1), as, add);
}
template <int HT, int NT, int GL, int NG, bool ACT, class ADD>
__device__ __forceinline__ void rw_gn_mish_half(f32x4 (&acc)[HT][NT], const float (&bias)[NT], const float (&gamma)[NT],
                                                const float (&beta)[NT], const float (&isc)[NT], float inv, const ActScale& as, ADD add,
                                                HalfStat* xch, int hf, int lane) {
  float k[NT];
  const float bsum4 = rw_gn_prologue<GL>(bias, isc, inv, k);
  const HalfStat own = rw_half_stat<HT, NT, GL, NG>(acc, bias, k, bsum4);
  xch[hf * 64 + lane] = own;
  __syncthreads();
  const HalfStat other = xch[(hf ^ 1) * 64 + lane];
  const GnStat st = hf ? gn_combine<NG>(other, own) : gn_combine<NG>(own, other);
  rw_gn_apply<HT, NT, ACT>(acc, bias, gamma, beta, k, st, as, add);
}
template <int MT, int NT>
__device__ __forceinline__ float rw_absmax(const f32x4 (&acc)[MT][NT]) {
  float m = 0.f;
#pragma unroll
  for (int mt = 0; mt < MT; ++mt)
#pragma unroll
    for (int t = 0; t < NT; ++t)
#pragma unroll
      for (int r = 0; r < 4; ++r) m = fmaxf(m, fabsf(acc[mt][t][r]));
  return wave_max(m);
}
template <class GEO, int MT>
__device__ __forceinline__ void rw_store2(char* vs, const f32x4 (&acc)[MT][2]) {
#pragma unroll
  for (int mt = 0; mt < MT; ++mt)
#pragma unroll
    for (int r = 0; r < 4; ++r) {
      const F16Pair f = f16_split2(acc[mt][0][r], acc[mt][1][r]);
      *reinterpret_cast<unsigned*>(vs + (mt * 16 + r) * 16) = f.hi;
      MMD_LO(*reinterpret_cast<unsigned*>(vs + GEO::PS + (mt * 16 + r) * 16) = f.lo;)
    }
}
__device__ __forceinline__ void wave_lds_fence() {
  __builtin_amdgcn_fence(__ATOMIC_ACQ_REL, "wavefront");
  __builtin_amdgcn_wave_barrier();
}

struct RwHalf { HalfStat* xch; int hf, lane; };
template <int GL, int NG, int MT, int NT, class ADDEND>
__device__ __forceinline__ void rw_gn(f32x4 (&acc)[MT][NT], const Epi<NT>& e, float inv, const ADDEND& addend) {
  const auto add = gn_addend(e, addend);
  rw_gn_mish_whole<MT, NT, GL, NG, decltype(add)::ACT>(acc, e.b, e.g, e.be, e.is, inv, add.as, add);
}
template <int GL, int NG, int HT, int NT, class ADDEND>
__device__ __forceinline__ void rw_gn(f32x4 (&acc)[HT][NT], const Epi<NT>& e, float inv, const ADDEND& addend, const RwHalf& h) {
  const auto add = gn_addend(e, addend);
  rw_gn_mish_half<HT, NT, GL, NG, decltype(add)::ACT>(acc, e.b, e.g, e.be, e.is, inv, add.as, add, h.xch, h.hf, h.lane);
}
template <int TPS>
__device__ __forceinline__ float sample_of(float act_s, int) { return act_s; }
template <int TPS, int M, int N>
__device__ __forceinline__ const f32x4 (&sample_of(const f32x4 (&t)[M][N], int sl))[TPS][N] { return sub_tile<TPS>(t, TPS * sl); }
template <int GL, int NG, int M, int NT, int S, class ADDEND>
__device__ __forceinline__ void rw_gn_samples(f32x4 (&acc)[M][NT], const Epi<NT>& e, const float (&inv)[S], const ADDEND& addend) {
  constexpr int TPS = M / S;
#pragma unroll
  for (int sl = 0; sl < S; ++sl) {
    const auto add = gn_addend(e, sample_of<TPS>(addend, sl));
    rw_gn_mish<TPS, NT, GL, NG, decltype(add)::ACT>(sub_tile<TPS>(acc, TPS * sl), e.b, e.g, e.be, e.is, inv[sl], add.as, add);
  }
}
template <class GEO>
__device__ __forceinline__ void rw_zero_halo(char* base, int rows, int lane, bool mine) {
  constexpr int KC = GEO::KC;
  if (mine && (16 * N_PIECES * KC >= 64 || lane < 16 * N_PIECES * KC)) {
    const int hr = lane & 3, blk = (lane >> 2) % (4 * KC), q = lane / (16 * KC);
    *reinterpret_cast<uint4*>(base + q * GEO::PS + (blk / KC) * GEO::G + (blk % KC) * GEO::BX + (hr < 2 ? hr : rows + hr) * 16) =
        make_uint4(0u, 0u, 0u, 0u);
  }
}
template <int K, int SLOT0, int NS>
__device__ __forceinline__ void pair_maxima_out(const f32x4 (&v)[NS][2], float* mx, int wave, int lane) {
  constexpr int SW = NS / 2;
  const int np = wave & 1, s0 = SW * (wave >> 1);
  float m2[2] = {0.f, 0.f};
#pragma unroll
  for (int sl = 0; sl < SW; ++sl) m2[sl] = rw_absmax(sub_tile<2>(v, 2 * sl));
  if (lane < K * SW) mx[(s0 + lane / K) * MX_SLOTS + SLOT0 + np + 2 * (lane & (K - 1))] = SW == 2 && lane / K ? m2[1] : m2[0];
}
template <int MT, int NT>
__device__ __forceinline__ float tail_epilogue(f32x4 (&y)[MT][NT], const float (&is)[NT], const float (&bt)[NT]) {
  float m = 0.f;
#pragma unroll
  for (int mt = 0; mt < MT; ++mt)
#pragma unroll
    for (int t = 0; t < NT; ++t)
#pragma unroll
      for (int r = 0; r < 4; ++r) {
        y[mt][t][r] = fmaf(y[mt][t][r], is[t], bt[t]);
        m = fmaxf(m, fabsf(y[mt][t][r]));
      }
  return wave_max(m);
}
template <int MT, int NT>
__device__ __forceinline__ float tail_up_epilogue(f32x4 (&e)[MT][NT], f32x4 (&o)[MT][NT], const float (&is0)[NT], const float (&is1)[NT],
                                                  const float (&bt)[NT]) {
  float m = 0.f;
#pragma unroll
  for (int mt = 0; mt < MT; ++mt)
#pragma unroll
    for (int t = 0; t < NT; ++t)
#pragma unroll
      for (int r = 0; r < 4; ++r) {
        e[mt][t][r] = fmaf(e[mt][t][r], is0[t], bt[t]);
        o[mt][t][r] = fmaf(o[mt][t][r], is1[t], bt[t]);
        m = fmaxf(m, fmaxf(fabsf(e[mt][t][r]), fabsf(o[mt][t][r])));
      }
  return wave_max(m);
}

template <int NFRAG>
__device__ __forceinline__ void stage_weights(const uint4* w, char* dst, int wave, int lane) {
  static_assert(NFRAG % 4 == 0, "fragments are dealt to the four waves");
  const uint4* src = w + lane;
  if constexpr (N_PIECES == 2) {
#pragma unroll
    for (int i = 0; i < NFRAG / 4; ++i) {
      const int f = wave + 4 * i;
      __builtin_amdgcn_global_load_lds((const __attribute__((address_space(1))) void*)(src + f * 64),
                                       (__attribute__((address_space(3))) void*)(dst + f * 1024), 16, 0, 0);
    }
  } else {
    constexpr int NF0 = NFRAG / 2;
#pragma unroll
    for (int i = 0; i < (NF0 + 3) / 4; ++i) {
      const int f = 2 * (wave + 4 * i);
      if (4 * i + 3 < NF0 || wave + 4 * i < NF0)
        __builtin_amdgcn_global_load_lds((const __attribute__((address_space(1))) void*)(src + f * 64),
                                         (__attribute__((address_space(3))) void*)(dst + f * 1024), 16, 0, 0);
    }
  }
}
__device__ __forceinline__ void staged_weights_landed() { asm volatile("s_waitcnt vmcnt(0)" ::: "memory"); }
constexpr int WBUF_BYTES = 20 * 1024;
__device__ __forceinline__ float half_sample_max(float* mx, int sp, int hf, int lane, float own) {
  if (lane < 4) mx[sp * MX_SLOTS + 4 * hf + lane] = own;
  __syncthreads();
  return mx_read(mx, sp);
}

struct D0 {
  using GW = RwGeo<32, 64>;
  static constexpr int XIN = 72 * 8;
  static constexpr int W_BYTES = GW::BYTES + 2 * XIN + 128;
  static_assert(4 * W_BYTES <= MX_OFF * 4, "four private slabs");
  static_assert(2 * W_BYTES + 2 * WBUF_BYTES <= MX_OFF * 4, "two samples' slabs + two weight buffers below the maxima");
  static_assert(GW::FRAGS5 * 2 * 1024 <= WBUF_BYTES, "a staged conv fits its buffer");
};
__device__ __forceinline__ float d0_stage_input(const float* in0, bool valid, size_t smp, int lane, char* xin, bool store) {
  float4 v = make_float4(0.f, 0.f, 0.f, 0.f);
  if (valid) v = *reinterpret_cast<const float4*>(in0 + (smp * 64 + lane) * 4);
  const DynScale ds = dyn_scale(wave_max(fmaxf(fmaxf(fabsf(v.x), fabsf(v.y)), fmaxf(fabsf(v.z), fabsf(v.w)))));
  const F16Pair p0 = f16_split2(v.x * ds.s, v.y * ds.s), p1 = f16_split2(v.z * ds.s, v.w * ds.s);
  if (store) {
    *reinterpret_cast<uint2*>(xin + (2 + lane) * 8) = make_uint2(p0.hi, p1.hi);
    MMD_LO(*reinterpret_cast<uint2*>(xin + D0::XIN + (2 + lane) * 8) = make_uint2(p0.lo, p1.lo);)
  }
  return ds.inv;
}
__device__ __forceinline__ void d0_zero_xin_halo(char* xin, int lane, bool mine) {
  if (mine && lane < 8 * N_PIECES) {
    const int row = (lane & 7) < 2 ? (lane & 7) : 64 + (lane & 7);
    *reinterpret_cast<uint2*>(xin + (lane >> 3) * D0::XIN + row * 8) = make_uint2(0u, 0u);
  }
}
__device__ __forceinline__ void d0_load_wa(const ChainArgs& a, int lane, u32x4 (&b)[2][2], u32x4 (&br)[2][2]) {
  const WTiles<2> wa = w_local(w_tiles<2>(a.r0.wa_bf, 2, 0, lane)), wr = w_local(w_tiles<2>(a.wres_bf, 2, 0, lane), wa);
#pragma unroll
  for (int t = 0; t < 2; ++t)
#pragma unroll
    for (int q = 0; q < 2; ++q) {
      b[t][q] = wa.frag(t, q);
      br[t][q] = wr.frag(t, q);
    }
}
template <int MT>
__device__ __forceinline__ void d0_conv_a(f32x4 (&acc)[MT][2], f32x4 (&res)[MT][2], const char* xin, int m0, int n, int g,
                                          const u32x4 (&b)[2][2], const u32x4 (&br)[2][2]) {
#pragma unroll
  for (int mt = 0; mt < MT; ++mt) {
    u32x4 af[2];
#pragma unroll
    for (int q = 0; q < 2; ++q) {
      const uint2* p = reinterpret_cast<const uint2*>(xin + q * D0::XIN + ((m0 + mt) * 16 + n + 2 * g) * 8);
      const uint2 lo = p[0], hi = p[1];
      af[q] = u32x4{lo.x, lo.y, hi.x, hi.y};
    }
#pragma unroll
    for (int t = 0; t < 2; ++t) {
      vb_three<true>(acc[mt][t], af, b[t]);
      vb_three<true>(res[mt][t], af, br[t]);
    }
  }
}
template <int MT>
__device__ __forceinline__ void d0_tail_store(char* lb, int smp, int m0, int n, int g, const f32x4 (&y)[MT][2], float so) {
  using GN = RlGeo<32>;
  char* xb = lb + (n >> 2) * GN::G + (smp * GN::RPS + 2 + 16 * m0 + 4 * g) * 16 + (n & 3) * 4;
#pragma unroll
  for (int mt = 0; mt < MT; ++mt)
#pragma unroll
    for (int r = 0; r < 4; ++r) {
      const F16Pair f = f16_split2(y[mt][0][r] * so, y[mt][1][r] * so);
      *reinterpret_cast<unsigned*>(xb + (16 * mt + r) * 16) = f.hi;
      MMD_LO(*reinterpret_cast<unsigned*>(xb + GN::PS + (16 * mt + r) * 16) = f.lo;)
    }
}

template <int NS>
__device__ __forceinline__ void chain_body_d0w(const ChainArgs& a, float* lds, int n0, int lane, int wave, int trb, int tb_off = 0) {
  using GW = D0::GW;
  char* const slab = reinterpret_cast<char*>(lds) + wave * D0::W_BYTES;
  char* const xin = slab + GW::BYTES;
  const int n = lane & 15, g = lane >> 4, c0 = 2 * n;
  const char* const va = slab + g * GW::G + n * 16;
  char* const vs = slab + (n >> 2) * GW::G + (2 + 4 * g) * 16 + (n & 3) * 4;
  TR(trb + 0);
  const float inv_in = d0_stage_input(a.in0, wave < NS && n0 + wave < a.n, n0 + wave, lane, xin, true);
  d0_zero_xin_halo(xin, lane, true);
  rw_zero_halo<GW>(slab, 64, lane, true);
  wave_lds_fence();
  f32x4 acc[4][2], res[4][2];
  const Epi<2> e0a = epi_a<2>(a.r0, tb_off, c0);
  const float br0[2] = {a.br[c0], a.br[c0 + 1]}, isr0[2] = {a.isr[c0], a.isr[c0 + 1]};
  {
    u32x4 b[2][2], br[2][2];
    d0_load_wa(a, lane, b, br);
    d0_conv_a<4>(acc, res, xin, 0, n, g, b, br);
  }
  u32x4 ring[5][2][2];
  auto preload = [&](const uint4* w) { rd_ring_load<GW, 2, 5>(ring, w_tiles<2>(w, GW::FRAGS5, 0, lane)); };
  auto conv = [&](const uint4* w) {
    const WTiles<2> wp = w_tiles<2>(w, GW::FRAGS5, 0, lane);
    rw_store2<GW, 4>(vs, acc);
    wave_lds_fence();
    rd_taps<GW, 2, 0, 5, true, false, 4, 5>(acc, res, va, wp, wp, ring);
    wave_lds_fence();
  };
  tile_finish_res(res, isr0, inv_in, br0);
  preload(a.r0.wb_bf);
  rw_gn<2, 256>(acc, e0a, inv_in, a.r0.act_a);
  TR(trb + 1);
  {
    const Epi<2> e = epi_b<2>(a.r0, c0);
    conv(a.r0.wb_bf);
    preload(a.ri[0].wa_bf);
    rw_gn<2, 256>(acc, e, 1.f, res);
  }
  TR(trb + 2);
  {
    const RtbPtrs& R = a.ri[0];
    tile_copy(res, acc);
    const DynScale ds = dyn_scale(rw_absmax(acc));
    tile_scale(acc, ds.s);
    const Epi<2> ea = epi_a<2>(R, tb_off, c0);
    conv(R.wa_bf);
    preload(R.wb_bf);
    rw_gn<2, 256>(acc, ea, ds.inv, R.act_a);
    TR(trb + 3);
    const Epi<2> eb = epi_b<2>(R, c0);
    conv(R.wb_bf);
    rw_gn<2, 256>(acc, eb, 1.f, res);
    TR(trb + 4);
  }
  {
    const DynScale ds = dyn_scale(rw_absmax(acc));
    tile_scale(acc, ds.s);
    const WTiles<2> wt = w_tiles<2>(a.wt_bf0, GW::FRAGS3, 0, lane);
    u32x4 ring3[3][2][2];
    const float bt[2] = {a.bt[c0], a.bt[c0 + 1]}, ist[2] = {a.ist0[c0] * ds.inv, a.ist0[c0 + 1] * ds.inv};
    rd_ring_load<GW, 2, 3>(ring3, wt);
    rw_store2<GW, 4>(vs, acc);
    wave_lds_fence();
    f32x4 y[2][2];
    rd_taps<Stride2<GW, 0, 2>, 2, 1, 3, true, false, 2, 3>(y, y, va + n * 16, wt, wt, ring3);
    const float mo = tail_epilogue(y, ist, bt);
    __syncthreads();
    if (lane < MX_SLOTS) (lds + MX_OFF)[wave * MX_SLOTS + lane] = mo;
    char* const lb = reinterpret_cast<char*>(lds);
    d0_tail_store<2>(lb, wave, 0, n, g, y, dyn_scale(mo).s);
    rw_zero_halo<RlGeo<32>>(lb + wave * RlGeo<32>::RPS * 16, 32, lane, true);
  }
  TR(trb + 5);
}

template <int NV>
__device__ __forceinline__ void chain_body_d0s(const ChainArgs& a, float* lds, int n0, int lane, int wave, int trb, int tb_off = 0) {
  using GW = D0::GW;
  const int sp = wave >> 1, hf = wave & 1;
  char* const slab = reinterpret_cast<char*>(lds) + sp * D0::W_BYTES;
  char* const xin = slab + GW::BYTES;
  float* const mx = lds + MX_OFF;
  const RwHalf half{reinterpret_cast<HalfStat*>(lds + PARK2_OFF) + sp * 128, hf, lane};
  static_assert(2 * 128 * sizeof(HalfStat) <= 3 * 256 * 16, "exchange area inside the parking area");
  char* const wb0 = reinterpret_cast<char*>(lds) + 2 * D0::W_BYTES;
  char* const wb1 = wb0 + WBUF_BYTES;
  stage_weights<2 * GW::FRAGS5>(a.r0.wb_bf, wb0, wave, lane);
  const int n = lane & 15, g = lane >> 4, c0 = 2 * n;
  const char* const va = slab + g * GW::G + (n + 32 * hf) * 16;
  char* const vs = slab + (n >> 2) * GW::G + (2 + 4 * g + 32 * hf) * 16 + (n & 3) * 4;
  TR(trb + 0);
  const float inv_in = d0_stage_input(a.in0, sp < NV && n0 + sp < a.n, n0 + sp, lane, xin, (lane >> 5) == hf);
  d0_zero_xin_halo(xin, lane, hf == 0);
  rw_zero_halo<GW>(slab, 64, lane, hf == 0);
  f32x4 acc[2][2], res[2][2];
  const Epi<2> e0a = epi_a<2>(a.r0, tb_off, c0);
  const float br0[2] = {a.br[c0], a.br[c0 + 1]}, isr0[2] = {a.isr[c0], a.isr[c0 + 1]};
  u32x4 b0[2][2], br[2][2];
  d0_load_wa(a, lane, b0, br);
  __syncthreads();
  d0_conv_a<2>(acc, res, xin, 2 * hf, n, g, b0, br);
  u32x4 ring[2][2][2];
  auto conv = [&](char* wb, auto next_frags, const uint4* w_next, char* wb_next, int tr = -1) {
    const WStaged<2> wp = w_staged<2>(wb, GW::FRAGS5, lane);
    if (tr >= 0) TR(tr);
    rw_store2<GW, 2>(vs, acc);
    if (tr >= 0) TR(tr + 1);
    staged_weights_landed();
    __syncthreads();
    if (tr >= 0) TR(tr + 2);
    if constexpr (decltype(next_frags)::value > 0) stage_weights<decltype(next_frags)::value>(w_next, wb_next, wave, lane);
    rd_ring_load<GW, 2, 2>(ring, wp);
    rd_taps<GW, 2, 0, 5, true, false, 2, 2>(acc, res, va, wp, wp, ring);
    if (tr >= 0) TR(tr + 3);
  };
  using F5 = std::integral_constant<int, 2 * GW::FRAGS5>;
  using F3 = std::integral_constant<int, 2 * GW::FRAGS3>;
  tile_finish_res(res, isr0, inv_in, br0);
  rw_gn<2, 256>(acc, e0a, inv_in, a.r0.act_a, half);
  TR(trb + 1);
  {
    const Epi<2> e = epi_b<2>(a.r0, c0);
    conv(wb0, F5{}, a.ri[0].wa_bf, wb1);
    rw_gn<2, 256>(acc, e, 1.f, res, half);
  }
  TR(trb + 2);
  {
    const RtbPtrs& R = a.ri[0];
    tile_copy(res, acc);
    const DynScale ds = dyn_scale(half_sample_max(mx, sp, hf, lane, rw_absmax(acc)));
    tile_scale(acc, ds.s);
    const Epi<2> ea = epi_a<2>(R, tb_off, c0);
    conv(wb1, F5{}, R.wb_bf, wb0, trb + 6);
    TR(trb + 10);
    rw_gn<2, 256>(acc, ea, ds.inv, R.act_a, half);
    TR(trb + 3);
    const Epi<2> eb = epi_b<2>(R, c0);
    conv(wb0, F3{}, a.wt_bf0, wb1);
    rw_gn<2, 256>(acc, eb, 1.f, res, half);
    TR(trb + 4);
  }
  {
    const DynScale ds = dyn_scale(half_sample_max(mx, sp, hf, lane, rw_absmax(acc)));
    tile_scale(acc, ds.s);
    const WStaged<2> wt = w_staged<2>(wb1, GW::FRAGS3, lane);
    const float bt[2] = {a.bt[c0], a.bt[c0 + 1]}, ist[2] = {a.ist0[c0] * ds.inv, a.ist0[c0 + 1] * ds.inv};
    rw_store2<GW, 2>(vs, acc);
    staged_weights_landed();
    __syncthreads();
    f32x4 y[1][2];
    rd_ring_load<GW, 2, 2>(ring, wt);
    rd_taps<Stride2<GW, 0, 2>, 2, 1, 3, true, false, 1, 2>(y, y, va + n * 16, wt, wt, ring);
    const float mo = tail_epilogue(y, ist, bt);
    const float so = dyn_scale(half_sample_max(mx, sp, hf, lane, mo)).s;
    char* const lb = reinterpret_cast<char*>(lds);
    d0_tail_store<1>(lb, sp, hf, n, g, y, so);
    rw_zero_halo<RlGeo<32>>(lb + sp * RlGeo<32>::RPS * 16, 32, lane, hf == 0);
  }
  TR(trb + 5);
}

template <int NS>
__device__ __forceinline__ void chain_body_d1d(const ChainArgs& a, float* lds, int lane, int wave, f32x4 (&skip)[NS][2], int trb, int tb_off = 0) {
  using GI = RlGeo<32>;
  using GH = RlGeo<64>;
  constexpr int H_OFF = GI::BYTES;
  static_assert(H_OFF + GH::BYTES <= MX_OFF * 4, "input slab + 64-channel slab");
  char* const lb = reinterpret_cast<char*>(lds);
  char* const slabH = lb + H_OFF;
  float* const mx = lds + MX_OFF;
  constexpr int SW = NS / 2;
  const int n = lane & 15, g = lane >> 4, np = wave & 1, sp = wave >> 1, s0 = SW * sp;
  const int c0 = 32 * np + 2 * n;
  const char* const vaI = lb + g * GI::G + (s0 * GI::RPS + n) * 16;
  const char* const vaH = slabH + g * GH::G + (s0 * GH::RPS + n) * 16;
  char* const vsH = slabH + (2 * np + (n >> 3)) * GH::G + ((n >> 2) & 1) * GH::BX + (s0 * GH::RPS + 2 + 4 * g) * 16 + (n & 3) * 4;
  auto wt2 = [&](const uint4* w, int frags) { return w_tiles<2>(w, frags, 2 * np, lane); };
  f32x4 acc[NS][2], res[NS][2];
  constexpr int RD1 = MMD_D1_RD;
  u32x4 ring[RD1][2][2];
  auto store_tile = [&]() {
#pragma unroll
    for (int m = 0; m < NS; ++m)
#pragma unroll
      for (int r = 0; r < 4; ++r) {
        const F16Pair f = f16_split2(acc[m][0][r], acc[m][1][r]);
        *reinterpret_cast<unsigned*>(vsH + (GH::tile_row(m) + r) * 16) = f.hi;
        MMD_LO(*reinterpret_cast<unsigned*>(vsH + GH::PS + (GH::tile_row(m) + r) * 16) = f.lo;)
      }
  };
  constexpr bool PF = ring_prefetch(NS);
  auto prefetch = [&](const uint4* w, int frags) {
    if constexpr (PF) rd_ring_load<GH, 2, RD1>(ring, wt2(w, frags));
  };
  auto conv = [&](const uint4* w, const uint4* w_next, int frags_next) {
    const WTiles<2> wp = wt2(w, GH::FRAGS5);
    if constexpr (!PF) rd_ring_load<GH, 2, RD1>(ring, wp);
    store_tile();
    __syncthreads();
    rd_taps<GH, 2, 0, 5, true, false, NS, RD1>(acc, acc, vaH, wp, wp, ring);
    prefetch(w_next, frags_next);
  };
  float one2[SW];
#pragma unroll
  for (int sl = 0; sl < SW; ++sl) one2[sl] = 1.f;

  {
    u32x4 ring5[5][2][2];
    const WTiles<2> wpa = wt2(a.r0.wa_bf, GI::FRAGS5), wpr = wt2(a.wres_bf, 2 * GI::KC);
    rd_ring_load<GI, 2, 5>(ring5, wpa);
    const Epi<2> e0a = epi_a<2>(a.r0, tb_off, c0);
    const float br[2] = {a.br[c0], a.br[c0 + 1]}, isr[2] = {a.isr[c0], a.isr[c0 + 1]};
    __syncthreads();
    TR(trb + 0);
    float inv_in[SW];
#pragma unroll
    for (int sl = 0; sl < SW; ++sl) inv_in[sl] = dyn_scale(mx_read(mx, s0 + sl)).inv;
    rd_zero_halo<GH>(slabH);
    rd_taps<GI, 2, 0, 5, true, true, NS, 5>(acc, res, vaI, wpa, wpr, ring5);
    tile_finish_res(res, isr, inv_in, br);
    prefetch(a.r0.wb_bf, GH::FRAGS5);
    rw_gn_samples<4, 256>(acc, e0a, inv_in, a.r0.act_a);
  }
  TR(trb + 1);
  {
    const Epi<2> e = epi_b<2>(a.r0, c0);
    conv(a.r0.wb_bf, a.ri[0].wa_bf, GH::FRAGS5);
    rw_gn_samples<4, 256>(acc, e, one2, res);
  }
  TR(trb + 2);
  {
    const RtbPtrs& R = a.ri[0];
    tile_copy(res, acc);
    pair_maxima_out<4, 0>(acc, mx, wave, lane);
    __syncthreads();
    float inv[SW];
    mx_scale_tile(mx, s0, acc, inv);
    const Epi<2> ea = epi_a<2>(R, tb_off, c0);
    conv(R.wa_bf, R.wb_bf, GH::FRAGS5);
    rw_gn_samples<4, 256>(acc, ea, inv, R.act_a);
    TR(trb + 3);
    __syncthreads();
    const Epi<2> eb = epi_b<2>(R, c0);
    conv(R.wb_bf, a.wt_bf0, GH::FRAGS3);
    rw_gn_samples<4, 256>(acc, eb, one2, res);
    TR(trb + 4);
    tile_copy(skip, acc);
  }
  {
    pair_maxima_out<4, 0>(acc, mx, wave, lane);
    __syncthreads();
    float inv[SW];
    mx_scale_tile(mx, s0, acc, inv);
    const WTiles<2> wt = wt2(a.wt_bf0, GH::FRAGS3);
    const float bt[2] = {a.bt[c0], a.bt[c0 + 1]}, ist[2] = {a.ist0[c0], a.ist0[c0 + 1]};
    if constexpr (!PF) rd_ring_load<GH, 2, RD1>(ring, wt);
    store_tile();
    __syncthreads();
    f32x4 y[2][2];
    rd_taps<Stride2<GH, SW == 2 ? GH::RPS : 0, 1>, 2, 1, 3, true, false, 2, RD1>(y, y, vaH + n * 16, wt, wt, ring);
    float m2[2] = {0.f, 0.f};
#pragma unroll
    for (int sl = 0; sl < SW; ++sl) {
      const float is[2] = {ist[0] * inv[sl], ist[1] * inv[sl]};
      m2[sl] = tail_epilogue(sub_tile<1>(y, sl), is, bt);
    }
    __syncthreads();
    if (lane < 4 * SW) mx[(s0 + (lane >> 2)) * MX_SLOTS + np + 2 * (lane & 3)] = (lane >> 2) ? m2[1] : m2[0];
    float* xb = lds + s0 * D2::XSS + (2 + 4 * g) * D2::XSTR + c0;
#pragma unroll
    for (int sl = 0; sl < SW; ++sl)
#pragma unroll
      for (int r = 0; r < 4; ++r)
        *reinterpret_cast<float2*>(xb + sl * D2::XSS + r * D2::XSTR) = make_float2(y[sl][0][r], y[sl][1][r]);
  }
  TR(trb + 5);
}

__device__ __forceinline__ float* park_slot(float* lds, int i) {
  return (i < 5 ? lds + i * 1024 : lds + PARK2_OFF + (i - 5) * 1024) + opaque_tid() * 4;
}
template <int NS>
__device__ __forceinline__ void park_tile(float* lds, const f32x4 (&t)[NS][2]) {
#pragma unroll
  for (int i = 0; i < 2 * NS; ++i) *reinterpret_cast<f32x4*>(park_slot(lds, i)) = t[i >> 1][i & 1];
}
template <int NS>
__device__ __forceinline__ void unpark_tile(float* lds, f32x4 (&t)[NS][2]) {
#pragma unroll
  for (int i = 0; i < 2 * NS; ++i) t[i >> 1][i & 1] = *reinterpret_cast<const f32x4*>(park_slot(lds, i));
}

template <int NS>
__device__ __forceinline__ void chain_body_d2d(const ChainArgs& a, float* lds, int lane, int wave, f32x4 (&acc)[NS][2],
                                               f32x4 (&mid)[NS][2], int trb, int tb_off = 0) {
  using G128 = RdGeo<128>;
  using G64 = RdGeo<64>;
  const int n = lane & 15, g = lane >> 4;
  const int c0 = 32 * wave + 2 * n;
  static_assert(D2::SLAB_OFF + G128::BYTES <= MX_OFF * 4, "x slab + Rd slab must fit below the maxima");
  static_assert(D2::SLAB_OFF >= 5 * 1024 * 4, "the dead x slab holds 5 of the 8 parked float4 per thread");
  char* const slab = reinterpret_cast<char*>(lds) + D2::SLAB_OFF;
  float* const mx = lds + MX_OFF;
  const char* const va128 = slab + g * G128::G + n * 16;
  const char* const va64 = slab + g * G64::G + n * 16;
  char* const vs = slab + wave * G128::G + (n >> 2) * G128::BX + (2 + 4 * g) * 16 + (n & 3) * 4;
  auto wt2 = [&](const uint4* w, int frags) { return w_tiles<2>(w, frags, 2 * wave, lane); };
  constexpr int RDD = MMD_D2_RD;
  u32x4 ring[RDD][2][2];
  const WTiles<2> wpa = wt2(a.r0.wa_bf, G64::FRAGS5), wpr = wt2(a.wres_bf, 2 * G64::KC);
  rd_ring_load<G64, 2, 2>(reinterpret_cast<u32x4(&)[2][2][2]>(ring), wpa);
  __syncthreads();
  TR(trb + 0);

  float one4[NS];
#pragma unroll
  for (int sm = 0; sm < NS; ++sm) one4[sm] = 1.f;
  auto gn_unparked = [&](const Epi<2>& e) {
    f32x4 res[NS][2];
    unpark_tile(lds, res);
    rd_gn<256>(acc, e, one4, res);
  };
  constexpr bool PF = ring_prefetch(NS);
  auto prefetch = [&](const uint4* w) {
    if constexpr (PF) rd_ring_load<G128, 2, RDD>(ring, wt2(w, G128::FRAGS5));
  };
  auto conv = [&](const uint4* w, const uint4* w_next) {
    const WTiles<2> wp = wt2(w, G128::FRAGS5);
    TR(trb + 10);
    if constexpr (!PF) rd_ring_load<G128, 2, RDD>(ring, wp);
    rd_store2<G128>(vs, acc);
    TR(trb + 11);
    __syncthreads();
    TR(trb + 12);
    rd_taps<G128, 2, 0, 5, true, false, NS, RDD>(acc, acc, va128, wp, wp, ring);
    if (w_next) prefetch(w_next);
    TR(trb + 13);
  };

  float inv_in[NS];
#pragma unroll
  for (int sm = 0; sm < NS; ++sm) inv_in[sm] = dyn_scale(mx_read(mx, sm)).inv;
  rd_zero_halo<G64>(slab);
  const Epi<2> e0a = epi_a<2>(a.r0, tb_off, c0);
  const float br[2] = {a.br[c0], a.br[c0 + 1]}, isr[2] = {a.isr[c0], a.isr[c0 + 1]};
  rowform_to_rd<D2::C0, D2::XSS, D2::XSTR, NS>(lds, slab, mx);
  __syncthreads();
  {
    f32x4 res[NS][2];
    rd_taps<G64, 2, 0, 5, true, true, NS, 2>(acc, res, va64, wpa, wpr, reinterpret_cast<u32x4(&)[2][2][2]>(ring));
    tile_finish_res(res, isr, inv_in, br);
    park_tile(lds, res);
  }
  prefetch(a.r0.wb_bf);
  rd_gn<256>(acc, e0a, inv_in, a.r0.act_a);
  TR(trb + 1);
  __syncthreads();
  rd_zero_halo<G128>(slab);
  {
    const Epi<2> e = epi_b<2>(a.r0, c0);
    conv(a.r0.wb_bf, D2::N_IDENT > 0 ? a.ri[0].wa_bf : nullptr);
    gn_unparked(e);
  }

#pragma unroll 1
  for (int k = 0; k < D2::N_IDENT; ++k) {
    const RtbPtrs& R = a.ri[k];
    park_tile(lds, acc);
    rd_dyn_out<2>(acc, mx, wave, lane, k == D2::MID_AFTER ? 1 : 0);
    __syncthreads();
    float inv[NS];
    mx_scale_tile(mx, 0, acc, inv);
    const Epi<2> ea = epi_a<2>(R, tb_off, c0);
    conv(R.wa_bf, R.wb_bf);
    rd_gn<256>(acc, ea, inv, R.act_a);
    __syncthreads();
    const Epi<2> eb = epi_b<2>(R, c0);
    conv(R.wb_bf, k + 1 < D2::N_IDENT ? a.ri[k + 1].wa_bf : nullptr);
    gn_unparked(eb);
    TR(trb + 18);
    if (D2::MID_AFTER == k + 1) tile_copy(mid, acc);
  }
  rd_dyn_out<2>(acc, mx, wave, lane, 2);
}

template <int NS, class STORE2>
__device__ __forceinline__ void chain_body_u0d(const ChainArgs& a, float* lds, int lane, int wave, f32x4 (&x0)[NS][2],
                                               f32x4 (&x1)[NS][2], STORE2 store2, char* slab128, f32x4 (&xe)[NS][1],
                                               f32x4 (&xo)[NS][1], int trb, int tb_off = 0) {
  using G128 = RdGeo<128>;
  using G64 = RdGeo<64>;
  const int n = lane & 15, g = lane >> 4, col = 16 * wave + n;
  char* const slab64 = reinterpret_cast<char*>(lds);
  static_assert(G64::BYTES <= MX_OFF * 4, "64-channel Rd slab");
  float* const mx = lds + MX_OFF;
  const char* const va128 = slab128 + g * G128::G + n * 16;
  const char* const va64 = slab64 + g * G64::G + n * 16;
  char* const vs64 = slab64 + wave * G64::G + (n >> 3) * G64::BX + (2 + 4 * g) * 16 + ((n & 7) >> 1) * 4;
  auto wt1 = [&](const uint4* w, int frags) { return w_tiles<1>(w, frags, wave, lane); };
  constexpr int RDU = MMD_U0_RD;
  u32x4 ringa[RDU][1][2];
  constexpr int RDC = MMD_U0C_RD;
  u32x4 ring[RDC][1][2];
  const WTiles<1> wp0 = wt1(a.r0.wa_bf, G128::FRAGS5), wp1 = wt1(a.wa0_c1_bf, G128::FRAGS5);
  const WTiles<1> wr0 = wt1(a.wres_bf, 2 * G128::KC), wr1 = wt1(a.wres_c1_bf, 2 * G128::KC);
  rd_ring_load<G128, 1, RDU>(ringa, wp0);
  __syncthreads();
  TR(trb + 0);

  f32x4 acc[NS][1], res[NS][1];
  float one4[NS];
#pragma unroll
  for (int sm = 0; sm < NS; ++sm) one4[sm] = 1.f;
  constexpr bool PF = ring_prefetch(NS);
  auto prefetch64 = [&](const uint4* w, int frags) {
    if constexpr (PF) rd_ring_load<G64, 1, RDC>(ring, wt1(w, frags));
  };
  auto conv64 = [&](const uint4* w, const uint4* w_next, int frags_next) {
    const WTiles<1> wp = wt1(w, G64::FRAGS5);
    if constexpr (!PF) rd_ring_load<G64, 1, RDC>(ring, wp);
    rd_store1<G64>(vs64, acc, lane);
    __syncthreads();
    rd_taps<G64, 1, 0, 5, true, false, NS, RDC>(acc, res, va64, wp, wp, ring);
    prefetch64(w_next, frags_next);
  };

  float inv_in[NS];
#pragma unroll
  for (int sm = 0; sm < NS; ++sm) {
    const DynScale ds = dyn_scale(max_nn(mx_read(mx + MX_REGION, sm), mx_read(mx + 2 * MX_REGION, sm)));
    inv_in[sm] = ds.inv;
    tile_scale(sub_tile<1>(x0, sm), ds.s);
    tile_scale(sub_tile<1>(x1, sm), ds.s);
  }
  const Epi<1> e0a = epi_a<1>(a.r0, tb_off, col);
  const float br[1] = {a.br[col]}, isr[1] = {a.isr[col]};
  store2(x0);
  TR(160);
  __syncthreads();
  TR(161);
  rd_taps<G128, 1, 0, 5, true, true, NS, RDU>(acc, res, va128, wp0, wr0, ringa);
  rd_ring_load<G128, 1, RDU>(ringa, wp1);
  TR(162);
  __syncthreads();
  store2(x1);
  TR(163);
  __syncthreads();
  TR(164);
  rd_taps<G128, 1, 0, 5, false, true, NS, RDU>(acc, res, va128, wp1, wr1, ringa);
  TR(165);
  tile_finish_res(res, isr, inv_in, br);
  prefetch64(a.r0.wb_bf, G64::FRAGS5);
  rd_gn<128>(acc, e0a, inv_in, a.r0.act_a);
  TR(trb + 1);
  __syncthreads();
  rd_zero_halo<G64>(slab64);
  {
    const Epi<1> e = epi_b<1>(a.r0, col);
    conv64(a.r0.wb_bf, a.ri[0].wa_bf, G64::FRAGS5);
    rd_gn<128>(acc, e, one4, res);
  }
  TR(trb + 4);
  {
    const RtbPtrs& R = a.ri[0];
    tile_copy(res, acc);
    rd_dyn_out<1>(acc, mx, wave, lane, 0);
    __syncthreads();
    float inv[NS];
    mx_scale_tile(mx, 0, acc, inv);
    const Epi<1> ea = epi_a<1>(R, tb_off, col);
    conv64(R.wa_bf, R.wb_bf, G64::FRAGS5);
    rd_gn<128>(acc, ea, inv, R.act_a);
    TR(trb + 5);
    __syncthreads();
    const Epi<1> eb = epi_b<1>(R, col);
    conv64(R.wb_bf, a.wt_bf0, 2 * G64::KC * 2);
    rd_gn<128>(acc, eb, one4, res);
    TR(trb + 6);
  }
  {
    rd_dyn_out<1>(acc, mx, wave, lane, 0);
    __syncthreads();
    float inv[NS];
    mx_scale_tile(mx, 0, acc, inv);
    const WTiles<1> wt0 = wt1(a.wt_bf0, 2 * G64::KC * 2), wt1p = wt1(a.wt_bf1, 2 * G64::KC * 2);
    const float bt[1] = {a.bt[col]}, is0 = a.ist0[col], is1 = a.ist1[col];
    if constexpr (!PF) rd_ring_load<G64, 1, RDC>(ring, wt0);
    rd_store1<G64>(vs64, acc, lane);
    __syncthreads();
    TR(trb + 7);
    rd_taps<G64, 1, 1, 2, true, false, NS, RDC>(xe, res, va64, wt0, wt0, ring);
    rd_ring_load<G64, 1, RDC>(ring, wt1p);
    rd_taps<G64, 1, 2, 2, true, false, NS, RDC>(xo, res, va64, wt1p, wt1p, ring);
#pragma unroll
    for (int sm = 0; sm < NS; ++sm) {
      const float s0[1] = {is0 * inv[sm]}, s1[1] = {is1 * inv[sm]};
      const float m = tail_up_epilogue(sub_tile<1>(xe, sm), sub_tile<1>(xo, sm), s0, s1, bt);
      if (lane == 0) mx[sm * MX_SLOTS + wave] = m;
    }
  }
}

struct U1 {
  using GA = RwGeo<64, 32>;
  using GB = RwGeo<32, 32>;
  using GF = RwGeo<32, 64>;
  static constexpr int W_BYTES = cmax(GA::BYTES, cmax(GB::BYTES, GF::BYTES)) + 128;
  static constexpr int RDA = 5;
  static constexpr int TF = 2 * (2 * GB::KC * 2);
  static_assert(4 * W_BYTES <= MX_OFF * 4, "four private slabs");
  static_assert(2 * W_BYTES + 2 * WBUF_BYTES <= MX_OFF * 4, "two samples' slabs + two weight buffers below the maxima");
  static_assert(GB::FRAGS5 * 2 * 1024 <= WBUF_BYTES && GF::FRAGS5 * 2 * 1024 <= WBUF_BYTES, "a staged conv fits its buffer");
};
__device__ __forceinline__ float lane_swap1(float v) {
  return __builtin_bit_cast(float, __builtin_amdgcn_update_dpp(0, __builtin_bit_cast(int, v), 0xB1, 0xf, 0xf, true));
}
template <int NS> struct U1Scales { float sc[NS]; DynScale skip[NS / 2]; };
template <int NS>
__device__ __forceinline__ U1Scales<NS> u1_input_scales(const float* mx, int wave) {
  U1Scales<NS> s;
#pragma unroll
  for (int sm = 0; sm < NS; ++sm) s.sc[sm] = dyn_scale(mx_read(mx, sm)).s;
#pragma unroll
  for (int sl = 0; sl < NS / 2; ++sl) s.skip[sl] = dyn_scale(mx_read(mx, NS / 2 * (wave >> 1) + sl));
  return s;
}
template <int NS>
__device__ __forceinline__ void u1_store_chunk0(char* lb, int wave, int n, int g, const f32x4 (&xe)[NS][1], const f32x4 (&xo)[NS][1],
                                                const float (&sc)[NS]) {
  using GA = U1::GA;
  const bool odd = n & 1;
  char* const d0 = lb + wave * GA::G + (n >> 3) * GA::BX + ((n & 7) >> 1) * 4 + 2 * 16 + (8 * g + (odd ? 1 : 0)) * 16;
#pragma unroll
  for (int sm = 0; sm < NS; ++sm)
#pragma unroll
    for (int r = 0; r < 4; ++r) {
      const float own = (odd ? xo[sm][0][r] : xe[sm][0][r]) * sc[sm];
      const float recv = lane_swap1((odd ? xe[sm][0][r] : xo[sm][0][r]) * sc[sm]);
      const F16Pair p = f16_split2(odd ? recv : own, odd ? own : recv);
      char* d = d0 + sm * U1::W_BYTES + 2 * r * 16;
      *reinterpret_cast<unsigned*>(d) = p.hi;
      MMD_LO(*reinterpret_cast<unsigned*>(d + GA::PS) = p.lo;)
    }
}
template <int NS>
__device__ __forceinline__ void u1_store_chunk1(char* lb, int wave, int n, int g, const f32x4 (&skip)[NS][2], const DynScale (&sc)[NS / 2]) {
  using GA = U1::GA;
  const int np = wave & 1, s0 = NS / 2 * (wave >> 1);
  char* const sdst = lb + (2 * np + (n >> 3)) * GA::G + ((n >> 2) & 1) * GA::BX + (n & 3) * 4 + (2 + 4 * g) * 16;
#pragma unroll
  for (int m = 0; m < NS; ++m)
#pragma unroll
    for (int r = 0; r < 4; ++r) {
      const F16Pair p = f16_split2(skip[m][0][r] * sc[m >> 1].s, skip[m][1][r] * sc[m >> 1].s);
      char* d = sdst + (s0 + (m >> 1)) * U1::W_BYTES + (16 * (m & 1) + r) * 16;
      *reinterpret_cast<unsigned*>(d) = p.hi;
      MMD_LO(*reinterpret_cast<unsigned*>(d + GA::PS) = p.lo;)
    }
}
template <int MT>
__device__ __forceinline__ void u1_tail_store(char* vsF, int m0, int g, const f32x4 (&e)[MT][2], const f32x4 (&o)[MT][2], float s) {
  using GF [[maybe_unused]] = U1::GF;
#pragma unroll
  for (int mt = 0; mt < MT; ++mt)
#pragma unroll
    for (int r = 0; r < 4; ++r) {
      const F16Pair pe = f16_split2(e[mt][0][r] * s, e[mt][1][r] * s), po = f16_split2(o[mt][0][r] * s, o[mt][1][r] * s);
      char* d = vsF + (2 + 32 * (m0 + mt) + 8 * g + 2 * r) * 16;
      *reinterpret_cast<unsigned*>(d) = pe.hi;
      MMD_LO(*reinterpret_cast<unsigned*>(d + GF::PS) = pe.lo;)
      *reinterpret_cast<unsigned*>(d + 16) = po.hi;
      MMD_LO(*reinterpret_cast<unsigned*>(d + 16 + GF::PS) = po.lo;)
    }
}
template <int MT>
__device__ __forceinline__ void u1_eps_to_slab(float* et, int m0, int n, int g, const f32x4 (&out)[MT][1], float s1, float b1) {
  if (n < 4) {
#pragma unroll
    for (int mt = 0; mt < MT; ++mt)
#pragma unroll
      for (int r = 0; r < 4; ++r) et[(16 * (m0 + mt) + 4 * g + r) * 4 + n] = fmaf(out[mt][0][r], s1, b1);
  }
}
template <int MT>
__device__ __forceinline__ void u1_store_out(float* eps, size_t smp, int m0, int n, int g, const f32x4 (&out)[MT][1], float s1, float b1) {
  float* dst = eps + (smp * 64 + 16 * m0 + 4 * g) * 4 + n;
#pragma unroll
  for (int mt = 0; mt < MT; ++mt)
#pragma unroll
    for (int r = 0; r < 4; ++r) dst[(16 * mt + r) * 4] = fmaf(out[mt][0][r], s1, b1);
}
__device__ __forceinline__ void fused_ddpm_row(const FusedStep& fs, const float* et, int smp, int lane) {
  const float4 e = *reinterpret_cast<const float4*>(et + lane * 4);
  const int traj = fs.traj0 + smp, robot = traj / fs.spr;
  const size_t idx = (size_t)traj * H + lane;
  float4 v = ddpm_posterior_mean(fs.x[idx], e, fs.a_t, fs.b_t, fs.c1, fs.c2);
  if (fs.do_noise)
    v = add_step_noise(v, fs.noise ? fs.noise[idx] : traj_normal4(fs.seed, fs.robot_seeds, fs.draw, fs.traj_base, idx, robot, fs.spr), fs.sigma,
                       fs.noise_std_extra);
  float4 hv;
  if (hard_row(fs.hard_rows, fs.n_hard, fs.hard, robot, lane, hv)) v = hv;
  fs.x[idx] = v;
  if (fs.chain) fs.chain[idx] = v;
}

template <int NS>
__device__ __forceinline__ void chain_body_u1w(const ChainArgs& a, const FinalArgs& f, const FusedStep& fs, float* lds, int n0, int lane_in, int wave,
                                               const f32x4 (&xe)[NS][1], const f32x4 (&xo)[NS][1], const f32x4 (&skip)[NS][2],
                                               int trb, int tb_off = 0) {
  int lane = lane_in;
  asm volatile("" : "+v"(lane));
  using GA = U1::GA;
  using GB = U1::GB;
  using GF = U1::GF;
  constexpr int RDA = U1::RDA;
  char* const lb = reinterpret_cast<char*>(lds);
  char* const slab = lb + wave * U1::W_BYTES;
  float* const mx = lds + MX_OFF;
  const int n = lane & 15, g = lane >> 4, c0 = 2 * n;
  auto wt2 = [&](const uint4* w, int frags) { return w_tiles<2>(w, frags, 0, lane); };
  const WTiles<2> wp0 = wt2(a.r0.wa_bf, GA::FRAGS5), wp1 = wt2(a.wa0_c1_bf, GA::FRAGS5);
  const WTiles<2> wr0 = wt2(a.wres_bf, 2 * GA::KC), wr1 = wt2(a.wres_c1_bf, 2 * GA::KC);
  u32x4 ring[RDA][2][2];
  rd_ring_load<GA, 2, RDA>(ring, wp0);
  pair_maxima_out<2, 4>(skip, mx, wave, lane);
  __syncthreads();
  TR(trb + 0);
  const U1Scales<NS> sc = u1_input_scales<NS>(mx, wave);
  const float inv_in = dyn_scale(mx_read(mx, wave)).inv;
  rw_zero_halo<GA>(slab, 32, lane, true);
  u1_store_chunk0(lb, wave, n, g, xe, xo, sc.sc);
  TR(trb + 6);
  __syncthreads();
  TR(trb + 7);
  const char* const vaA = slab + g * GA::G + n * 16;
  f32x4 acc[2][2], res[2][2];
  rd_taps<GA, 2, 0, 5, true, true, 2, RDA>(acc, res, vaA, wp0, wr0, ring);
  rd_ring_load<GA, 2, RDA>(ring, wp1);
  TR(trb + 8);
  __syncthreads();
  u1_store_chunk1(lb, wave, n, g, skip, sc.skip);
  __syncthreads();
  TR(trb + 10);
  const Epi<2> e0a = epi_a<2>(a.r0, tb_off, c0);
  const float br[2] = {a.br[c0], a.br[c0 + 1]}, isr[2] = {a.isr[c0], a.isr[c0 + 1]};
  rd_taps<GA, 2, 0, 5, false, true, 2, RDA>(acc, res, vaA, wp1, wr1, ring);
  TR(trb + 11);
  const char* const vaB = slab + g * GB::G + n * 16;
  char* const vsB = slab + (n >> 2) * GB::G + (2 + 4 * g) * 16 + (n & 3) * 4;
  u32x4 ring5[5][2][2];
  auto preload = [&](const uint4* w) { rd_ring_load<GB, 2, 5>(ring5, wt2(w, GB::FRAGS5)); };
  preload(a.r0.wb_bf);
  auto conv = [&](const uint4* w) {
    const WTiles<2> wp = wt2(w, GB::FRAGS5);
    rw_store2<GB, 2>(vsB, acc);
    wave_lds_fence();
    rd_taps<GB, 2, 0, 5, true, false, 2, 5>(acc, res, vaB, wp, wp, ring5);
    wave_lds_fence();
  };
  tile_finish_res(res, isr, inv_in, br);
  rw_gn<2, 128>(acc, e0a, inv_in, a.r0.act_a);
  TR(trb + 1);
  wave_lds_fence();
  rw_zero_halo<GB>(slab, 32, lane, true);
  {
    const Epi<2> e = epi_b<2>(a.r0, c0);
    conv(a.r0.wb_bf);
    preload(a.ri[0].wa_bf);
    rw_gn<2, 128>(acc, e, 1.f, res);
  }
  TR(trb + 2);
  {
    const RtbPtrs& R = a.ri[0];
    tile_copy(res, acc);
    const DynScale ds = dyn_scale(rw_absmax(acc));
    tile_scale(acc, ds.s);
    const Epi<2> ea = epi_a<2>(R, tb_off, c0);
    conv(R.wa_bf);
    preload(R.wb_bf);
    rw_gn<2, 128>(acc, ea, ds.inv, R.act_a);
    TR(trb + 3);
    const Epi<2> eb = epi_b<2>(R, c0);
    conv(R.wb_bf);
    rw_gn<2, 128>(acc, eb, 1.f, res);
    TR(trb + 4);
  }
  const char* const vaF = slab + g * GF::G + n * 16;
  char* const vsF = slab + (n >> 2) * GF::G + (n & 3) * 4;
  f32x4 y[4][2];
  float inv_f;
  {
    const DynScale ds = dyn_scale(rw_absmax(acc));
    tile_scale(acc, ds.s);
    const WTiles<2> wt0 = wt2(a.wt_bf0, 2 * GB::KC * 2), wt1 = wt2(a.wt_bf1, 2 * GB::KC * 2);
    u32x4 ring2[2][2][2];
    const float bt[2] = {a.bt[c0], a.bt[c0 + 1]};
    const float is0[2] = {a.ist0[c0] * ds.inv, a.ist0[c0 + 1] * ds.inv}, is1[2] = {a.ist1[c0] * ds.inv, a.ist1[c0 + 1] * ds.inv};
    rd_ring_load<GB, 2, 2>(ring2, wt0);
    rw_store2<GB, 2>(vsB, acc);
    wave_lds_fence();
    f32x4 e[2][2], o[2][2];
    rd_taps<GB, 2, 1, 2, true, false, 2, 2>(e, res, vaB, wt0, wt0, ring2);
    rd_ring_load<GB, 2, 2>(ring2, wt1);
    rd_taps<GB, 2, 2, 2, true, false, 2, 2>(o, res, vaB, wt1, wt1, ring2);
    const DynScale df = dyn_scale(tail_up_epilogue(e, o, is0, is1, bt));
    inv_f = df.inv;
    wave_lds_fence();
    rw_zero_halo<GF>(slab, 64, lane, true);
    u1_tail_store<2>(vsF, 0, g, e, o, df.s);
  }
  TR(trb + 5);
  {
    const WTiles<2> wf = wt2(f.w5, GF::FRAGS5);
    rd_ring_load<GF, 2, 5>(ring5, wf);
    const WTiles<1> w1 = w_tiles<1>(f.w1_bf, 2 * GF::KC, 0, lane);
    u32x4 ring1[1][1][2];
    rd_ring_load<GF, 1, 1>(ring1, w1);
    const Epi<2> ef = epi_load<2>(f.bias, f.gamma, f.beta, nullptr, f.isc, c0);
    const float b1 = f.w1_bias[n & 3], s1 = f.is1[n & 3];
    wave_lds_fence();
    rd_taps<GF, 2, 0, 5, true, false, 4, 5>(y, y, vaF, wf, wf, ring5);
    rw_gn_mish_whole<4, 2, 2, 256, true>(y, ef.b, ef.g, ef.be, ef.is, inv_f, act_scale(f.act), [](int, int, int) { return 0.f; });
    wave_lds_fence();
    rw_store2<GF, 4>(vsF + (2 + 4 * g) * 16, y);
    wave_lds_fence();
    f32x4 out[4][1];
    rd_taps<GF, 1, 2, 1, true, false, 4, 1>(out, out, vaF, w1, w1, ring1);
    auto valid = [&] { return wave < NS && n0 + wave < a.n; };
    if (fs.enabled) {
      float* const et = reinterpret_cast<float*>(slab);
      wave_lds_fence();
      u1_eps_to_slab<4>(et, 0, n, g, out, s1, b1);
      wave_lds_fence();
      if (valid()) fused_ddpm_row(fs, et, n0 + wave, lane);
    } else if (n < 4 && valid()) {
      u1_store_out<4>(f.out, n0 + wave, 0, n, g, out, s1, b1);
    }
  }
}

template <int NV>
__device__ __forceinline__ void chain_body_u1s(const ChainArgs& a, const FinalArgs& f, const FusedStep& fs, float* lds, int n0, int lane_in, int wave,
                                               const f32x4 (&xe)[2][1], const f32x4 (&xo)[2][1], const f32x4 (&skip)[2][2], int trb, int tb_off = 0) {
  int lane = lane_in;
  asm volatile("" : "+v"(lane));
  using GA = U1::GA;
  using GB = U1::GB;
  using GF = U1::GF;
  constexpr int RDA = U1::RDA, TF = U1::TF;
  char* const lb = reinterpret_cast<char*>(lds);
  const int sp = wave >> 1, hf = wave & 1;
  char* const slab = lb + sp * U1::W_BYTES;
  float* const mx = lds + MX_OFF;
  const RwHalf half{reinterpret_cast<HalfStat*>(lds + PARK2_OFF) + sp * 128, hf, lane};
  const int n = lane & 15, g = lane >> 4, c0 = 2 * n;
  auto wt2 = [&](const uint4* w, int frags) { return w_tiles<2>(w, frags, 0, lane); };
  const WTiles<2> wp0 = wt2(a.r0.wa_bf, GA::FRAGS5), wp1 = wt2(a.wa0_c1_bf, GA::FRAGS5);
  const WTiles<2> wr0 = wt2(a.wres_bf, 2 * GA::KC), wr1 = wt2(a.wres_c1_bf, 2 * GA::KC);
  u32x4 ring[RDA][2][2];
  rd_ring_load<GA, 2, RDA>(ring, wp0);
  pair_maxima_out<2, 4>(skip, mx, wave, lane);
  __syncthreads();
  TR(trb + 0);
  char* const wb0 = lb + 2 * U1::W_BYTES;
  char* const wb1 = wb0 + WBUF_BYTES;
  stage_weights<2 * GB::FRAGS5>(a.r0.wb_bf, wb0, wave, lane);
  const U1Scales<2> sc = u1_input_scales<2>(mx, wave);
  const float inv_in = sc.skip[0].inv;
  rw_zero_halo<GA>(slab, 32, lane, hf == 0);
  u1_store_chunk0(lb, wave, n, g, xe, xo, sc.sc);
  TR(trb + 6);
  __syncthreads();
  TR(trb + 7);
  const char* const vaA = slab + g * GA::G + (n + 16 * hf) * 16;
  f32x4 acc[1][2], res[1][2];
  rd_taps<GA, 2, 0, 5, true, true, 1, RDA>(acc, res, vaA, wp0, wr0, ring);
  rd_ring_load<GA, 2, RDA>(ring, wp1);
  TR(trb + 8);
  __syncthreads();
  u1_store_chunk1(lb, wave, n, g, skip, sc.skip);
  __syncthreads();
  TR(trb + 10);
  const Epi<2> e0a = epi_a<2>(a.r0, tb_off, c0);
  const float br[2] = {a.br[c0], a.br[c0 + 1]}, isr[2] = {a.isr[c0], a.isr[c0 + 1]};
  rd_taps<GA, 2, 0, 5, false, true, 1, RDA>(acc, res, vaA, wp1, wr1, ring);
  TR(trb + 11);
  const char* const vaB = slab + g * GB::G + (n + 16 * hf) * 16;
  char* const vsB = slab + (n >> 2) * GB::G + (2 + 4 * g + 16 * hf) * 16 + (n & 3) * 4;
  u32x4 ring2[2][2][2];
  auto conv = [&](char* wb, auto stage_next) {
    const WStaged<2> wp = w_staged<2>(wb, GB::FRAGS5, lane);
    rw_store2<GB, 1>(vsB, acc);
    staged_weights_landed();
    __syncthreads();
    stage_next();
    rd_ring_load<GB, 2, 2>(ring2, wp);
    rd_taps<GB, 2, 0, 5, true, false, 1, 2>(acc, res, vaB, wp, wp, ring2);
  };
  tile_finish_res(res, isr, inv_in, br);
  rw_gn<2, 128>(acc, e0a, inv_in, a.r0.act_a, half);
  TR(trb + 1);
  rw_zero_halo<GB>(slab, 32, lane, hf == 0);
  {
    const Epi<2> e = epi_b<2>(a.r0, c0);
    conv(wb0, [&] { stage_weights<2 * GB::FRAGS5>(a.ri[0].wa_bf, wb1, wave, lane); });
    rw_gn<2, 128>(acc, e, 1.f, res, half);
  }
  TR(trb + 2);
  {
    const RtbPtrs& R = a.ri[0];
    tile_copy(res, acc);
    const DynScale ds = dyn_scale(half_sample_max(mx, sp, hf, lane, rw_absmax(acc)));
    tile_scale(acc, ds.s);
    const Epi<2> ea = epi_a<2>(R, tb_off, c0);
    conv(wb1, [&] { stage_weights<2 * GB::FRAGS5>(R.wb_bf, wb0, wave, lane); });
    rw_gn<2, 128>(acc, ea, ds.inv, R.act_a, half);
    TR(trb + 3);
    const Epi<2> eb = epi_b<2>(R, c0);
    conv(wb0, [&] {
      stage_weights<TF>(a.wt_bf0, wb1, wave, lane);
      stage_weights<TF>(a.wt_bf1, wb1 + TF * 1024, wave, lane);
    });
    rw_gn<2, 128>(acc, eb, 1.f, res, half);
    TR(trb + 4);
  }
  const char* const vaF = slab + g * GF::G + (n + 32 * hf) * 16;
  char* const vsF = slab + (n >> 2) * GF::G + (n & 3) * 4;
  f32x4 y[2][2];
  float inv_f;
  {
    const DynScale ds = dyn_scale(half_sample_max(mx, sp, hf, lane, rw_absmax(acc)));
    tile_scale(acc, ds.s);
    const WStaged<2> wt0 = w_staged<2>(wb1, TF / 2, lane), wt1 = w_staged<2>(wb1 + TF * 1024, TF / 2, lane);
    const float bt[2] = {a.bt[c0], a.bt[c0 + 1]};
    const float is0[2] = {a.ist0[c0] * ds.inv, a.ist0[c0 + 1] * ds.inv}, is1[2] = {a.ist1[c0] * ds.inv, a.ist1[c0 + 1] * ds.inv};
    rw_store2<GB, 1>(vsB, acc);
    staged_weights_landed();
    __syncthreads();
    stage_weights<2 * GF::FRAGS5>(f.w5, wb0, wave, lane);
    f32x4 e[1][2], o[1][2];
    rd_ring_load<GB, 2, 2>(ring2, wt0);
    rd_taps<GB, 2, 1, 2, true, false, 1, 2>(e, res, vaB, wt0, wt0, ring2);
    rd_ring_load<GB, 2, 2>(ring2, wt1);
    rd_taps<GB, 2, 2, 2, true, false, 1, 2>(o, res, vaB, wt1, wt1, ring2);
    const float m = tail_up_epilogue(e, o, is0, is1, bt);
    const DynScale df = dyn_scale(half_sample_max(mx, sp, hf, lane, m));
    inv_f = df.inv;
    rw_zero_halo<GF>(slab, 64, lane, hf == 0);
    u1_tail_store<1>(vsF, hf, g, e, o, df.s);
  }
  TR(trb + 5);
  {
    const WStaged<2> wf = w_staged<2>(wb0, GF::FRAGS5, lane);
    const WTiles<1> w1 = w_tiles<1>(f.w1_bf, 2 * GF::KC, 0, lane);
    u32x4 ring1[1][1][2];
    rd_ring_load<GF, 1, 1>(ring1, w1);
    const Epi<2> ef = epi_load<2>(f.bias, f.gamma, f.beta, nullptr, f.isc, c0);
    const float b1 = f.w1_bias[n & 3], s1 = f.is1[n & 3];
    staged_weights_landed();
    __syncthreads();
    rd_ring_load<GF, 2, 2>(ring2, wf);
    rd_taps<GF, 2, 0, 5, true, false, 2, 2>(y, y, vaF, wf, wf, ring2);
    rw_gn_mish_half<2, 2, 2, 256, true>(y, ef.b, ef.g, ef.be, ef.is, inv_f, act_scale(f.act), [](int, int, int) { return 0.f; }, half.xch, hf, lane);
    rw_store2<GF, 2>(vsF + (2 + 4 * g + 32 * hf) * 16, y);
    wave_lds_fence();
    f32x4 out[2][1];
    rd_taps<GF, 1, 2, 1, true, false, 2, 1>(out, out, vaF, w1, w1, ring1);
    auto valid = [&] { return sp < NV && n0 + sp < a.n; };
    if (fs.enabled) {
      float* const et = reinterpret_cast<float*>(slab);
      __syncthreads();
      u1_eps_to_slab<2>(et, 2 * hf, n, g, out, s1, b1);
      __syncthreads();
      if (hf == 0 && valid()) fused_ddpm_row(fs, et, n0 + sp, lane);
    } else if (n < 4 && valid()) {
      u1_store_out<2>(f.out, n0 + sp, 2 * hf, n, g, out, s1, b1);
    }
  }
}

struct UnetArgs {
  ChainArgs c[5];
  FinalArgs fin;
  int n;
  FusedStep fs;
};

template <int NS>
__device__ __forceinline__ void unet_forward_body(const UnetArgs& a, const FusedStep& fs, int tb_off, float* lds, int n0, int lane, int wave) {
  constexpr int NP = NS == 1 ? 2 : NS;
  f32x4 skip1[NP][2], skip2[NS][2], xe[NP][1], xo[NP][1];
  if constexpr (NS == 1) {
#pragma unroll
    for (int r = 0; r < 4; ++r) xe[1][0][r] = xo[1][0][r] = 0.f;
  }
  if constexpr (NS <= 2) chain_body_d0s<NS>(a.c[0], lds, n0, lane, wave, 0, tb_off);
  else chain_body_d0w<NS>(a.c[0], lds, n0, lane, wave, 0, tb_off);
  chain_body_d1d<NP>(a.c[1], lds, lane, wave, skip1, 40, tb_off);
  f32x4 mid_out[NS][2];
  chain_body_d2d<NS>(a.c[2], lds, lane, wave, mid_out, skip2, 80, tb_off);
  TR(130);
  {
    using G128 = RdGeo<128>;
    char* const slab128 = reinterpret_cast<char*>(lds) + D2::SLAB_OFF;
    char* const vs = slab128 + wave * G128::G + ((lane & 15) >> 2) * G128::BX + (2 + 4 * (lane >> 4)) * 16 + (lane & 3) * 4;
    chain_body_u0d<NS>(a.c[3], lds, lane, wave, mid_out, skip2, [&](const f32x4 (&t)[NS][2]) { rd_store2<G128>(vs, t); }, slab128,
                       sub_tile<NS>(xe, 0), sub_tile<NS>(xo, 0), 136, tb_off);
  }
  TR(131);
  if constexpr (NS <= 2) chain_body_u1s<NS>(a.c[4], a.fin, fs, lds, n0, lane, wave, xe, xo, skip1, 146, tb_off);
  else chain_body_u1w<NS>(a.c[4], a.fin, fs, lds, n0, lane, wave, xe, xo, skip1, 146, tb_off);
  TR(133);
}

template <int NS>
__global__ __launch_bounds__(256) __attribute__((amdgpu_waves_per_eu(2, 2))) void unet_kernel(UnetArgs a) {
  __shared__ __attribute__((aligned(16))) float lds[UNET_LDS_FLOATS];
  const int lane = threadIdx.x & 63;
  const int wave = __builtin_amdgcn_readfirstlane(threadIdx.x >> 6);
  unet_forward_body<NS>(a, a.fs, 0, lds, blockIdx.x * NS, lane, wave);
}

static_assert(sizeof(UnetArgs) <= PERSIST_TABLE_BYTES - PERSIST_ARGS_OFF, "the argument block fits its workspace region");
template <int NS>
__global__ __launch_bounds__(256) __attribute__((amdgpu_waves_per_eu(2, 2))) void unet_persist_kernel(const UnetArgs* ap, const FusedStep* steps,
                                                                                                     int n_steps, int tb_total) {
  __shared__ __attribute__((aligned(16))) float lds[UNET_LDS_FLOATS];
  const int lane = threadIdx.x & 63;
  const int wave = __builtin_amdgcn_readfirstlane(threadIdx.x >> 6);
  typedef const __attribute__((address_space(4))) UnetArgs* ConstArgs;
  typedef const __attribute__((address_space(4))) FusedStep* ConstStep;
  for (int s = 0; s < n_steps; ++s) {
    unsigned long long pa = reinterpret_cast<unsigned long long>(ap), ps = reinterpret_cast<unsigned long long>(steps + s);
    asm volatile("" : "+s"(pa), "+s"(ps));
    const UnetArgs& a = *(const UnetArgs*)(ConstArgs)pa;
    const FusedStep& fs = *(const FusedStep*)(ConstStep)ps;
    int lane_s = lane;
    asm volatile("" : "+v"(lane_s));
    unet_forward_body<NS>(a, fs, fs.t_row * tb_total, lds, blockIdx.x * NS, lane_s, wave);
    __threadfence_block();
    __syncthreads();
  }
}

#ifdef MMD_UNET_F16
}
#endif
}
```

Baseline: 97810.

## Batch cross-row reductions with permlane swaps and emit f16 split residual directly

```diff
diff --git a/include/mmd_amd_debug.h b/include/mmd_amd_debug.h
--- a/include/mmd_amd_debug.h
+++ b/include/mmd_amd_debug.h
@@ -37,6 +37,10 @@
                               uint64_t seed, uint32_t draw_index, void* workspace_dev, size_t workspace_bytes,
                               float* mu_dev, float* guide_chain_dev, uint32_t* trace_dev, void* stream);
 
+int mmd_debug_f16_split(const float* in_dev, uint16_t* hi_dev, uint16_t* lo_dev, int n, void* stream);
+
+int mmd_debug_rows_allreduce(const float* in_dev, float* sum_dev, float* max_dev, int ns, void* stream);
+
 #ifdef __cplusplus
 }
 #endif
diff --git a/mmd_amd/_lib.py b/mmd_amd/_lib.py
--- a/mmd_amd/_lib.py
+++ b/mmd_amd/_lib.py
@@ -1,5 +1,6 @@
 import ctypes as C
 import os
+import sys
 
 _HERE = os.path.dirname(os.path.abspath(__file__))
 LIB_PATH = os.path.join(_HERE, "lib", "libmmd_amd.so")
@@ -192,12 +193,24 @@
     "mmd_debug_ddpm_step_trace": (C.c_int, [C.c_void_p, C.POINTER(SamplerDesc), C.POINTER(GuideDesc), C.c_void_p, C.c_void_p,
                                             C.c_int, C.c_int, C.c_int, C.c_void_p, C.c_uint64, C.c_uint32, C.c_void_p, C.c_size_t,
                                             C.c_void_p, C.c_void_p, C.c_void_p, C.c_void_p]),
+    "mmd_debug_f16_split": (C.c_int, [C.c_void_p, C.c_void_p, C.c_void_p, C.c_int, C.c_void_p]),
+    "mmd_debug_rows_allreduce": (C.c_int, [C.c_void_p, C.c_void_p, C.c_void_p, C.c_int, C.c_void_p]),
 }
 TRACE_WORDS = 12
 
 EXPORTED_SYMBOLS = tuple(_SIGNATURES)
 DEBUG_SYMBOLS = tuple(_DEBUG_SIGNATURES)
 _lib = None
+
+
+def use_library(path):
+    global LIB_PATH
+    assert _lib is None, "use_library() comes before the first load()"
+    LIB_PATH = os.path.abspath(path)
+    other = C.CDLL(LIB_PATH)
+    for name in [n for n in _DEBUG_SIGNATURES if not hasattr(other, n)]:
+        print(f"mmd_amd: {LIB_PATH} has no {name}", file=sys.stderr)
+        del _DEBUG_SIGNATURES[name]
 
 
 def load():
diff --git a/mmd_amd/csrc/f16x2.h b/mmd_amd/csrc/f16x2.h
--- a/mmd_amd/csrc/f16x2.h
+++ b/mmd_amd/csrc/f16x2.h
@@ -25,11 +25,18 @@
 __device__ __forceinline__ F16Pair f16_split2(float v0, float v1) {
   const f16x2 h = __builtin_convertvector(f32x2{v0, v1}, f16x2);
   const unsigned hb = __builtin_bit_cast(unsigned, h);
+#ifdef MMD_SPLIT_CVT
   float d0, d1;
   asm("v_fma_mix_f32 %0, %1, -1.0, %2 op_sel_hi:[1,0,0]" : "=v"(d0) : "v"(hb), "v"(v0));
   asm("v_fma_mix_f32 %0, %1, -1.0, %2 op_sel:[1,0,0] op_sel_hi:[1,0,0]" : "=v"(d1) : "v"(hb), "v"(v1));
   const f16x2 l = __builtin_convertvector(f32x2{d0, d1}, f16x2);
   return F16Pair{hb, __builtin_bit_cast(unsigned, l)};
+#else
+  unsigned lo;
+  asm("v_fma_mixlo_f16 %0, %1, -1.0, %2 op_sel_hi:[1,0,0]" : "=v"(lo) : "v"(hb), "v"(v0));
+  asm("v_fma_mixhi_f16 %0, %1, -1.0, %2 op_sel:[1,0,0] op_sel_hi:[1,0,0]" : "+v"(lo) : "v"(hb), "v"(v1));
+  return F16Pair{hb, lo};
+#endif
 }
 __device__ __forceinline__ f32x4 mfma_h(const u32x4& a, const u32x4& b, const f32x4& c) {
   return __builtin_amdgcn_mfma_f32_16x16x32_f16(__builtin_bit_cast(f16x8, a), __builtin_bit_cast(f16x8, b), c, 0, 0, 0);
diff --git a/mmd_amd/csrc/unet.hip b/mmd_amd/csrc/unet.hip
--- a/mmd_amd/csrc/unet.hip
+++ b/mmd_amd/csrc/unet.hip
@@ -53,6 +53,23 @@
 
 static inline bool fused_config(int uid, int n_levels) { return uid == 32 && n_levels == 3; }
 
+__global__ void debug_f16_split_kernel(const float* in, uint16_t* hi, uint16_t* lo, int n) {
+  for (int i = threadIdx.x; 2 * i + 1 < n; i += blockDim.x) {
+    const F16Pair f = f16_split2(in[2 * i], in[2 * i + 1]);
+    hi[2 * i] = (uint16_t)f.hi, hi[2 * i + 1] = (uint16_t)(f.hi >> 16);
+    lo[2 * i] = (uint16_t)f.lo, lo[2 * i + 1] = (uint16_t)(f.lo >> 16);
+  }
+}
+template <int NS>
+__global__ void debug_rows_allreduce_kernel(const float* in, float* sum, float* mx) {
+  float s[NS], m[NS];
+#pragma unroll
+  for (int i = 0; i < NS; ++i) s[i] = m[i] = in[i * 64 + threadIdx.x];
+  rows_allreduce<RowsAdd>(s);
+  rows_allreduce<RowsMaxNN>(m);
+#pragma unroll
+  for (int i = 0; i < NS; ++i) sum[i * 64 + threadIdx.x] = s[i], mx[i * 64 + threadIdx.x] = m[i];
+}
 void launch_time_table(const TimeArgs& a, int T, hipStream_t st) { hipLaunchKernelGGL(time_table_kernel, dim3(T), dim3(128), 0, st, a); }
 
 static size_t pack_im2col4(std::vector<float>& blob, const float* w, int cout, bool is_res, const std::vector<float>& sc) {
@@ -487,6 +504,23 @@
 
 int mmd_unet_precision(mmd_unet_t u) { return u ? u->precision : -1; }
 
+int mmd_debug_f16_split(const float* in, uint16_t* hi, uint16_t* lo, int n, void* stream) {
+  MMD_REQUIRE(in && hi && lo, "mmd_debug_f16_split: NULL argument");
+  MMD_REQUIRE(n >= 2 && n % 2 == 0, "mmd_debug_f16_split: n = %d is not a positive even count", n);
+  hipLaunchKernelGGL(debug_f16_split_kernel, dim3(1), dim3(256), 0, (hipStream_t)stream, in, hi, lo, n);
+  MMD_HIP_CHECK(hipGetLastError());
+  return 0;
+}
+int mmd_debug_rows_allreduce(const float* in, float* sum, float* mx, int ns, void* stream) {
+  MMD_REQUIRE(in && sum && mx, "mmd_debug_rows_allreduce: NULL argument");
+  MMD_REQUIRE(ns == 1 || ns == 2 || ns == 4, "mmd_debug_rows_allreduce: ns = %d (1, 2 or 4)", ns);
+  if (ns == 1) hipLaunchKernelGGL(debug_rows_allreduce_kernel<1>, dim3(1), dim3(64), 0, (hipStream_t)stream, in, sum, mx);
+  else if (ns == 2) hipLaunchKernelGGL(debug_rows_allreduce_kernel<2>, dim3(1), dim3(64), 0, (hipStream_t)stream, in, sum, mx);
+  else hipLaunchKernelGGL(debug_rows_allreduce_kernel<4>, dim3(1), dim3(64), 0, (hipStream_t)stream, in, sum, mx);
+  MMD_HIP_CHECK(hipGetLastError());
+  return 0;
+}
+
 size_t mmd_unet_weight_bytes(mmd_unet_t u) {
   if (!u) return 0;
   return u->layered ? layered_weight_bytes(u->layered) : u->blob_bytes;
diff --git a/mmd_amd/csrc/unet_kernel.h b/mmd_amd/csrc/unet_kernel.h
--- a/mmd_amd/csrc/unet_kernel.h
+++ b/mmd_amd/csrc/unet_kernel.h
@@ -84,21 +84,68 @@
 __device__ __forceinline__ float max_xor16(float v) { const RowPair r = rows_xor16(v); return max_nn(r.a, r.b); }
 __device__ __forceinline__ float max_xor32(float v) { const RowPair r = rows_xor32(v); return max_nn(r.a, r.b); }
 
+__device__ __forceinline__ RowPair rows_swap16(float x, float y) {
+  const auto r = __builtin_amdgcn_permlane16_swap(__builtin_bit_cast(unsigned, x), __builtin_bit_cast(unsigned, y), false, false);
+  return RowPair{__builtin_bit_cast(float, (unsigned)r[0]), __builtin_bit_cast(float, (unsigned)r[1])};
+}
+__device__ __forceinline__ RowPair rows_swap32(float x, float y) {
+  const auto r = __builtin_amdgcn_permlane32_swap(__builtin_bit_cast(unsigned, x), __builtin_bit_cast(unsigned, y), false, false);
+  return RowPair{__builtin_bit_cast(float, (unsigned)r[0]), __builtin_bit_cast(float, (unsigned)r[1])};
+}
+struct RowsAdd { static __device__ __forceinline__ float op(const RowPair& r) { return r.a + r.b; } };
+struct RowsMaxNN { static __device__ __forceinline__ float op(const RowPair& r) { return max_nn(r.a, r.b); } };
+template <class OP, int N>
+__device__ __forceinline__ void rows_allreduce(float (&v)[N]) {
+  constexpr int N4 = N / 4 * 4, N2 = N4 + (N - N4) / 2 * 2;
+#pragma unroll
+  for (int i = 0; i < N4; i += 4) {
+    const float p = OP::op(rows_swap16(v[i], v[i + 1])), q = OP::op(rows_swap16(v[i + 2], v[i + 3]));
+    const float t = OP::op(rows_swap32(p, q));
+    const RowPair e = rows_xor16(t);
+    const RowPair a = rows_xor32(e.a), b = rows_xor32(e.b);
+    v[i] = a.a, v[i + 1] = b.a, v[i + 2] = a.b, v[i + 3] = b.b;
+  }
+#pragma unroll
+  for (int i = N4; i < N2; i += 2) {
+    const float p = OP::op(rows_swap16(v[i], v[i + 1]));
+    const float t = OP::op(rows_xor32(p));
+    const RowPair e = rows_xor16(t);
+    v[i] = e.a, v[i + 1] = e.b;
+  }
+#pragma unroll
+  for (int i = N2; i < N; ++i) v[i] = OP::op(rows_xor32(OP::op(rows_xor16(v[i]))));
+}
+
 template <int CTRL>
 __device__ __forceinline__ float dpp_max(float v) {
   return max_nn(v, __builtin_bit_cast(float, __builtin_amdgcn_update_dpp(0, __builtin_bit_cast(int, v), CTRL, 0xF, 0xF, true)));
 }
+template <int CTRL, int N>
+__device__ __forceinline__ void dpp_max_n(float (&v)[N]) {
+#pragma unroll
+  for (int i = 0; i < N; ++i) v[i] = dpp_max<CTRL>(v[i]);
+}
+template <int N>
+__device__ __forceinline__ void row_max16_n(float (&v)[N]) {
+  dpp_max_n<0xB1>(v);
+  dpp_max_n<0x4E>(v);
+  dpp_max_n<0x141>(v);
+  dpp_max_n<0x140>(v);
+}
+template <int N>
+__device__ __forceinline__ void wave_max_n(float (&v)[N]) {
+  row_max16_n(v);
+  rows_allreduce<RowsMaxNN>(v);
+}
 __device__ __forceinline__ float row_max16(float v) {
-  v = dpp_max<0xB1>(v);
-  v = dpp_max<0x4E>(v);
-  v = dpp_max<0x141>(v);
-  v = dpp_max<0x140>(v);
-  return v;
+  float a[1] = {v};
+  row_max16_n(a);
+  return a[0];
 }
 __device__ __forceinline__ float wave_max(float v) {
-  v = row_max16(v);
-  v = max_xor16(v);
-  return max_xor32(v);
+  float a[1] = {v};
+  wave_max_n(a);
+  return a[0];
 }
 constexpr int MX_SLOTS = 8;
 constexpr int MX_REGION = 4 * MX_SLOTS;
@@ -265,6 +312,17 @@
 __device__ __forceinline__ f32x4 (&sub_tile(f32x4 (&t)[M][N], int m0))[MS][N] { return reinterpret_cast<f32x4(&)[MS][N]>(t[m0]); }
 template <int MS, int M, int N>
 __device__ __forceinline__ const f32x4 (&sub_tile(const f32x4 (&t)[M][N], int m0))[MS][N] { return reinterpret_cast<const f32x4(&)[MS][N]>(t[m0]); }
+template <int MT, int NT>
+__device__ __forceinline__ float tile_absmax(const f32x4 (&acc)[MT][NT]) {
+  float m = 0.f;
+#pragma unroll
+  for (int mt = 0; mt < MT; ++mt)
+#pragma unroll
+    for (int t = 0; t < NT; ++t)
+#pragma unroll
+      for (int r = 0; r < 4; ++r) m = fmaxf(m, fabsf(acc[mt][t][r]));
+  return m;
+}
 
 template <int NT> struct AddTimeBias {
   static constexpr bool ACT = true;
@@ -289,13 +347,23 @@
 template <int MT, int NT>
 __device__ __forceinline__ AddResidual<MT, NT> gn_addend(const Epi<NT>&, const f32x4 (&res)[MT][NT]) { return AddResidual<MT, NT>{res, ActScale{}}; }
 
+template <int CTRL, int N>
+__device__ __forceinline__ void dpp_add_n(float (&v)[N]) {
+#pragma unroll
+  for (int i = 0; i < N; ++i) v[i] = dpp_add<CTRL>(v[i]);
+}
+template <int CPG, int N>
+__device__ __forceinline__ void group_colsum_n(float (&v)[N]) {
+  dpp_add_n<0xB1>(v);
+  dpp_add_n<0x4E>(v);
+  if constexpr (CPG >= 8) dpp_add_n<0x141>(v);
+  if constexpr (CPG >= 16) dpp_add_n<0x140>(v);
+}
 template <int CPG>
 __device__ __forceinline__ float group_colsum(float v) {
-  v = dpp_add<0xB1>(v);
-  v = dpp_add<0x4E>(v);
-  if constexpr (CPG >= 8) v = dpp_add<0x141>(v);
-  if constexpr (CPG >= 16) v = dpp_add<0x140>(v);
-  return v;
+  float a[1] = {v};
+  group_colsum_n<CPG>(a);
+  return a[0];
 }
 
 
@@ -430,12 +498,10 @@
       k[sm][t] = isc[t] * inv[sm];
       v = fmaf((acc[sm][t][0] + acc[sm][t][1]) + (acc[sm][t][2] + acc[sm][t][3]), k[sm][t], v);
     }
-    sum[sm] = group_colsum<8>(v);
-  }
-#pragma unroll
-  for (int sm = 0; sm < NS; ++sm) sum[sm] = add_xor16(sum[sm]);
-#pragma unroll
-  for (int sm = 0; sm < NS; ++sm) sum[sm] = add_xor32(sum[sm]);
+    sum[sm] = v;
+  }
+  group_colsum_n<8>(sum);
+  rows_allreduce<RowsAdd>(sum);
 #pragma unroll
   for (int sm = 0; sm < NS; ++sm) {
     const float mean = fmaf(sum[sm], inv_n, bmean);
@@ -449,12 +515,10 @@
         v = fmaf(d, d, v);
       }
     }
-    sq[sm] = group_colsum<8>(v);
-  }
-#pragma unroll
-  for (int sm = 0; sm < NS; ++sm) sq[sm] = add_xor16(sq[sm]);
-#pragma unroll
-  for (int sm = 0; sm < NS; ++sm) sq[sm] = add_xor32(sq[sm]);
+    sq[sm] = v;
+  }
+  group_colsum_n<8>(sq);
+  rows_allreduce<RowsAdd>(sq);
 #pragma unroll
   for (int sm = 0; sm < NS; ++sm) {
     const float rstd = __builtin_amdgcn_rsqf(fmaf(sq[sm], inv_n, 1e-5f));
@@ -478,18 +542,16 @@
 }
 template <int NT, int NS>
 __device__ __forceinline__ void rd_dyn_out(const f32x4 (&acc)[NS][NT], float* mx, int wave, int lane, int region2) {
+  float m[NS];
+#pragma unroll
+  for (int sm = 0; sm < NS; ++sm) m[sm] = tile_absmax(sub_tile<1>(acc, sm));
+  row_max16_n(m);
 #pragma unroll
   for (int sm = 0; sm < NS; ++sm) {
-    float m = 0.f;
-#pragma unroll
-    for (int t = 0; t < NT; ++t)
-#pragma unroll
-      for (int r = 0; r < 4; ++r) m = fmaxf(m, fabsf(acc[sm][t][r]));
-    m = row_max16(m);
-    m = max_xor16(m);
+    m[sm] = max_xor16(m[sm]);
     if ((lane & 31) == 0) {
-      mx[sm * MX_SLOTS + 2 * wave + (lane >> 5)] = m;
-      if (region2) mx[region2 * MX_REGION + sm * MX_SLOTS + 2 * wave + (lane >> 5)] = m;
+      mx[sm * MX_SLOTS + 2 * wave + (lane >> 5)] = m[sm];
+      if (region2) mx[region2 * MX_REGION + sm * MX_SLOTS + 2 * wave + (lane >> 5)] = m[sm];
     }
   }
 }
@@ -572,86 +634,114 @@
 template <class GEO, int SROWS, int TILES_PER_SAMPLE> struct Stride2 : GEO {
   static constexpr int tile_row(int m) { return (m / TILES_PER_SAMPLE) * SROWS + (m % TILES_PER_SAMPLE) * 32; }
 };
-__device__ __forceinline__ float wave_sum_rows(float v) {
-  v = add_xor16(v);
-  v = add_xor32(v);
-  return v;
+template <int GL, int N>
+__device__ __forceinline__ void rw_gsum_n(float (&v)[N]) {
+  dpp_add_n<0xB1>(v);
+  if constexpr (GL >= 4) dpp_add_n<0x4E>(v);
+  if constexpr (GL >= 8) dpp_add_n<0x141>(v);
+  rows_allreduce<RowsAdd>(v);
 }
 template <int GL>
 __device__ __forceinline__ float rw_gsum(float v) {
-  v = dpp_add<0xB1>(v);
-  if constexpr (GL >= 4) v = dpp_add<0x4E>(v);
-  if constexpr (GL >= 8) v = dpp_add<0x141>(v);
-  return wave_sum_rows(v);
-}
-template <int MT, int NT, int GL, int NG, bool ACT, class ADD>
-__device__ __forceinline__ void rw_gn_mish(f32x4 (&acc)[MT][NT], const float (&bias)[NT], const float (&gamma)[NT],
-                                           const float (&beta)[NT], const float (&isc)[NT], float inv, const ActScale& as, ADD add) {
+  float a[1] = {v};
+  rw_gsum_n<GL>(a);
+  return a[0];
+}
+template <int S, int MT, int NT, int GL, int NG, class ADDS>
+__device__ __forceinline__ void rw_gn_mish(f32x4 (&acc)[S * MT][NT], const float (&bias)[NT], const float (&gamma)[NT],
+                                           const float (&beta)[NT], const float (&isc)[NT], const float (&inv)[S], ADDS adds) {
   constexpr float inv_n = 1.f / (float)NG;
-  float k[NT], bsum = 0.f, v = 0.f;
-#pragma unroll
-  for (int t = 0; t < NT; ++t) {
-    k[t] = isc[t] * inv;
-    bsum += bias[t];
-    float st = 0.f;
-#pragma unroll
-    for (int mt = 0; mt < MT; ++mt) st += (acc[mt][t][0] + acc[mt][t][1]) + (acc[mt][t][2] + acc[mt][t][3]);
-    v = fmaf(st, k[t], v);
-  }
-  const float mean = (rw_gsum<GL>(v) + rw_gsum<GL>(bsum) * (float)(4 * MT)) * inv_n;
-  float dm[NT], q = 0.f;
-#pragma unroll
-  for (int t = 0; t < NT; ++t) {
-    dm[t] = mean - bias[t];
-#pragma unroll
-    for (int mt = 0; mt < MT; ++mt)
-#pragma unroll
-      for (int r = 0; r < 4; ++r) {
-        const float d = fmaf(acc[mt][t][r], k[t], -dm[t]);
-        q = fmaf(d, d, q);
-      }
-  }
-  const float rstd = __builtin_amdgcn_rsqf(fmaf(rw_gsum<GL>(q), inv_n, 1e-5f));
-#pragma unroll
-  for (int t = 0; t < NT; ++t) {
-    GnCoef cf = gn_coef(dm[t], rstd, gamma[t], beta[t]);
-    cf.sa *= k[t];
-#pragma unroll
-    for (int mt = 0; mt < MT; ++mt)
-#pragma unroll
-      for (int r = 0; r < 4; r += 2) {
-        const f32x2_t o = gn_mish2<ACT>(f32x2_t{acc[mt][t][r], acc[mt][t][r + 1]}, cf, f32x2_t{add(mt, t, r), add(mt, t, r + 1)}, as);
-        acc[mt][t][r] = o.x;
-        acc[mt][t][r + 1] = o.y;
-      }
+  constexpr bool ACT = decltype(adds(0))::ACT;
+  float k[S][NT], red[S + 1], bsum = 0.f;
+#pragma unroll
+  for (int t = 0; t < NT; ++t) bsum += bias[t];
+#pragma unroll
+  for (int sl = 0; sl < S; ++sl) {
+    float v = 0.f;
+#pragma unroll
+    for (int t = 0; t < NT; ++t) {
+      k[sl][t] = isc[t] * inv[sl];
+      float st = 0.f;
+#pragma unroll
+      for (int mt = 0; mt < MT; ++mt) st += (acc[MT * sl + mt][t][0] + acc[MT * sl + mt][t][1]) + (acc[MT * sl + mt][t][2] + acc[MT * sl + mt][t][3]);
+      v = fmaf(st, k[sl][t], v);
+    }
+    red[sl] = v;
+  }
+  red[S] = bsum;
+  rw_gsum_n<GL>(red);
+  float dm[S][NT], q[S];
+#pragma unroll
+  for (int sl = 0; sl < S; ++sl) {
+    const float mean = (red[sl] + red[S] * (float)(4 * MT)) * inv_n;
+    q[sl] = 0.f;
+#pragma unroll
+    for (int t = 0; t < NT; ++t) {
+      dm[sl][t] = mean - bias[t];
+#pragma unroll
+      for (int mt = 0; mt < MT; ++mt)
+#pragma unroll
+        for (int r = 0; r < 4; ++r) {
+          const float d = fmaf(acc[MT * sl + mt][t][r], k[sl][t], -dm[sl][t]);
+          q[sl] = fmaf(d, d, q[sl]);
+        }
+    }
+  }
+  rw_gsum_n<GL>(q);
+#pragma unroll
+  for (int sl = 0; sl < S; ++sl) {
+    const float rstd = __builtin_amdgcn_rsqf(fmaf(q[sl], inv_n, 1e-5f));
+    const auto add = adds(sl);
+#pragma unroll
+    for (int t = 0; t < NT; ++t) {
+      GnCoef cf = gn_coef(dm[sl][t], rstd, gamma[t], beta[t]);
+      cf.sa *= k[sl][t];
+#pragma unroll
+      for (int mt = 0; mt < MT; ++mt)
+#pragma unroll
+        for (int r = 0; r < 4; r += 2) {
+          const f32x2_t o = gn_mish2<ACT>(f32x2_t{acc[MT * sl + mt][t][r], acc[MT * sl + mt][t][r + 1]}, cf, f32x2_t{add(mt, t, r), add(mt, t, r + 1)}, add.as);
+          acc[MT * sl + mt][t][r] = o.x;
+          acc[MT * sl + mt][t][r + 1] = o.y;
+        }
+    }
   }
 }
 struct HalfStat { float mean, m2; };
-template <int HT, int NT, int GL, int NG>
-__device__ __forceinline__ HalfStat rw_half_stat(const f32x4 (&acc)[HT][NT], const float (&bias)[NT], const float (&k)[NT], float bsum4) {
-  float v = 0.f;
-#pragma unroll
-  for (int t = 0; t < NT; ++t) {
-    float st = (acc[0][t][0] + acc[0][t][1]) + (acc[0][t][2] + acc[0][t][3]);
-    if constexpr (HT == 2) st += (acc[1][t][0] + acc[1][t][1]) + (acc[1][t][2] + acc[1][t][3]);
-    v = fmaf(st, k[t], v);
-  }
-  HalfStat h;
-  h.mean = (rw_gsum<GL>(v) + bsum4 * (float)(4 * HT)) * (2.f / (float)NG);
-  float q = 0.f;
-#pragma unroll
-  for (int t = 0; t < NT; ++t) {
-    const float dm = h.mean - bias[t];
-#pragma unroll
-    for (int mt = 0; mt < HT; ++mt)
-#pragma unroll
-      for (int r = 0; r < 4; ++r) {
-        const float d = fmaf(acc[mt][t][r], k[t], -dm);
-        q = fmaf(d, d, q);
-      }
-  }
-  h.m2 = rw_gsum<GL>(q);
-  return h;
+template <int NH, int HT, int NT, int GL, int NG>
+__device__ __forceinline__ void rw_half_stats(const f32x4 (&acc)[NH * HT][NT], const float (&bias)[NT], const float (&k)[NT], float bsum4,
+                                              HalfStat (&h)[NH]) {
+  float v[NH], q[NH];
+#pragma unroll
+  for (int hf = 0; hf < NH; ++hf) {
+    v[hf] = 0.f;
+#pragma unroll
+    for (int t = 0; t < NT; ++t) {
+      float st = (acc[HT * hf][t][0] + acc[HT * hf][t][1]) + (acc[HT * hf][t][2] + acc[HT * hf][t][3]);
+      if constexpr (HT == 2) st += (acc[HT * hf + 1][t][0] + acc[HT * hf + 1][t][1]) + (acc[HT * hf + 1][t][2] + acc[HT * hf + 1][t][3]);
+      v[hf] = fmaf(st, k[t], v[hf]);
+    }
+  }
+  rw_gsum_n<GL>(v);
+#pragma unroll
+  for (int hf = 0; hf < NH; ++hf) {
+    h[hf].mean = (v[hf] + bsum4 * (float)(4 * HT)) * (2.f / (float)NG);
+    q[hf] = 0.f;
+#pragma unroll
+    for (int t = 0; t < NT; ++t) {
+      const float dm = h[hf].mean - bias[t];
+#pragma unroll
+      for (int mt = 0; mt < HT; ++mt)
+#pragma unroll
+        for (int r = 0; r < 4; ++r) {
+          const float d = fmaf(acc[HT * hf + mt][t][r], k[t], -dm);
+          q[hf] = fmaf(d, d, q[hf]);
+        }
+    }
+  }
+  rw_gsum_n<GL>(q);
+#pragma unroll
+  for (int hf = 0; hf < NH; ++hf) h[hf].m2 = q[hf];
 }
 struct GnStat { float mean, rstd; };
 template <int NG>
@@ -694,9 +784,9 @@
   static_assert(MT == 2 || MT == 4, "two halves of one or two M tiles");
   float k[NT];
   const float bsum4 = rw_gn_prologue<GL>(bias, isc, inv, k);
-  const HalfStat h0 = rw_half_stat<HT, NT, GL, NG>(sub_tile<HT>(acc, 0), bias, k, bsum4);
-  const HalfStat h1 = rw_half_stat<HT, NT, GL, NG>(sub_tile<HT>(acc, HT), bias, k, bsum4);
-  rw_gn_apply<MT, NT, ACT>(acc, bias, gamma, beta, k, gn_combine<NG>(h0, h1), as, add);
+  HalfStat h[2];
+  rw_half_stats<2, HT, NT, GL, NG>(acc, bias, k, bsum4, h);
+  rw_gn_apply<MT, NT, ACT>(acc, bias, gamma, beta, k, gn_combine<NG>(h[0], h[1]), as, add);
 }
 template <int HT, int NT, int GL, int NG, bool ACT, class ADD>
 __device__ __forceinline__ void rw_gn_mish_half(f32x4 (&acc)[HT][NT], const float (&bias)[NT], const float (&gamma)[NT],
@@ -704,7 +794,9 @@
                                                 HalfStat* xch, int hf, int lane) {
   float k[NT];
   const float bsum4 = rw_gn_prologue<GL>(bias, isc, inv, k);
-  const HalfStat own = rw_half_stat<HT, NT, GL, NG>(acc, bias, k, bsum4);
+  HalfStat h[1];
+  rw_half_stats<1, HT, NT, GL, NG>(acc, bias, k, bsum4, h);
+  const HalfStat own = h[0];
   xch[hf * 64 + lane] = own;
   __syncthreads();
   const HalfStat other = xch[(hf ^ 1) * 64 + lane];
@@ -712,16 +804,7 @@
   rw_gn_apply<HT, NT, ACT>(acc, bias, gamma, beta, k, st, as, add);
 }
 template <int MT, int NT>
-__device__ __forceinline__ float rw_absmax(const f32x4 (&acc)[MT][NT]) {
-  float m = 0.f;
-#pragma unroll
-  for (int mt = 0; mt < MT; ++mt)
-#pragma unroll
-    for (int t = 0; t < NT; ++t)
-#pragma unroll
-      for (int r = 0; r < 4; ++r) m = fmaxf(m, fabsf(acc[mt][t][r]));
-  return wave_max(m);
-}
+__device__ __forceinline__ float rw_absmax(const f32x4 (&acc)[MT][NT]) { return wave_max(tile_absmax(acc)); }
 template <class GEO, int MT>
 __device__ __forceinline__ void rw_store2(char* vs, const f32x4 (&acc)[MT][2]) {
 #pragma unroll
@@ -756,11 +839,7 @@
 template <int GL, int NG, int M, int NT, int S, class ADDEND>
 __device__ __forceinline__ void rw_gn_samples(f32x4 (&acc)[M][NT], const Epi<NT>& e, const float (&inv)[S], const ADDEND& addend) {
   constexpr int TPS = M / S;
-#pragma unroll
-  for (int sl = 0; sl < S; ++sl) {
-    const auto add = gn_addend(e, sample_of<TPS>(addend, sl));
-    rw_gn_mish<TPS, NT, GL, NG, decltype(add)::ACT>(sub_tile<TPS>(acc, TPS * sl), e.b, e.g, e.be, e.is, inv[sl], add.as, add);
-  }
+  rw_gn_mish<S, TPS, NT, GL, NG>(acc, e.b, e.g, e.be, e.is, inv, [&](int sl) { return gn_addend(e, sample_of<TPS>(addend, sl)); });
 }
 template <class GEO>
 __device__ __forceinline__ void rw_zero_halo(char* base, int rows, int lane, bool mine) {
@@ -775,10 +854,11 @@
 __device__ __forceinline__ void pair_maxima_out(const f32x4 (&v)[NS][2], float* mx, int wave, int lane) {
   constexpr int SW = NS / 2;
   const int np = wave & 1, s0 = SW * (wave >> 1);
-  float m2[2] = {0.f, 0.f};
-#pragma unroll
-  for (int sl = 0; sl < SW; ++sl) m2[sl] = rw_absmax(sub_tile<2>(v, 2 * sl));
-  if (lane < K * SW) mx[(s0 + lane / K) * MX_SLOTS + SLOT0 + np + 2 * (lane & (K - 1))] = SW == 2 && lane / K ? m2[1] : m2[0];
+  float m2[SW];
+#pragma unroll
+  for (int sl = 0; sl < SW; ++sl) m2[sl] = tile_absmax(sub_tile<2>(v, 2 * sl));
+  wave_max_n(m2);
+  if (lane < K * SW) mx[(s0 + lane / K) * MX_SLOTS + SLOT0 + np + 2 * (lane & (K - 1))] = SW == 2 && lane / K ? m2[SW - 1] : m2[0];
 }
 template <int MT, int NT>
 __device__ __forceinline__ float tail_epilogue(f32x4 (&y)[MT][NT], const float (&is)[NT], const float (&bt)[NT]) {
@@ -792,7 +872,7 @@
         y[mt][t][r] = fmaf(y[mt][t][r], is[t], bt[t]);
         m = fmaxf(m, fabsf(y[mt][t][r]));
       }
-  return wave_max(m);
+  return m;
 }
 template <int MT, int NT>
 __device__ __forceinline__ float tail_up_epilogue(f32x4 (&e)[MT][NT], f32x4 (&o)[MT][NT], const float (&is0)[NT], const float (&is1)[NT],
@@ -808,7 +888,7 @@
         o[mt][t][r] = fmaf(o[mt][t][r], is1[t], bt[t]);
         m = fmaxf(m, fmaxf(fabsf(e[mt][t][r]), fabsf(o[mt][t][r])));
       }
-  return wave_max(m);
+  return m;
 }
 
 template <int NFRAG>
@@ -976,7 +1056,7 @@
     wave_lds_fence();
     f32x4 y[2][2];
     rd_taps<Stride2<GW, 0, 2>, 2, 1, 3, true, false, 2, 3>(y, y, va + n * 16, wt, wt, ring3);
-    const float mo = tail_epilogue(y, ist, bt);
+    const float mo = wave_max(tail_epilogue(y, ist, bt));
     __syncthreads();
     if (lane < MX_SLOTS) (lds + MX_OFF)[wave * MX_SLOTS + lane] = mo;
     char* const lb = reinterpret_cast<char*>(lds);
@@ -1063,7 +1143,7 @@
     f32x4 y[1][2];
     rd_ring_load<GW, 2, 2>(ring, wt);
     rd_taps<Stride2<GW, 0, 2>, 2, 1, 3, true, false, 1, 2>(y, y, va + n * 16, wt, wt, ring);
-    const float mo = tail_epilogue(y, ist, bt);
+    const float mo = wave_max(tail_epilogue(y, ist, bt));
     const float so = dyn_scale(half_sample_max(mx, sp, hf, lane, mo)).s;
     char* const lb = reinterpret_cast<char*>(lds);
     d0_tail_store<1>(lb, sp, hf, n, g, y, so);
@@ -1171,14 +1251,15 @@
     __syncthreads();
     f32x4 y[2][2];
     rd_taps<Stride2<GH, SW == 2 ? GH::RPS : 0, 1>, 2, 1, 3, true, false, 2, RD1>(y, y, vaH + n * 16, wt, wt, ring);
-    float m2[2] = {0.f, 0.f};
+    float m2[SW];
 #pragma unroll
     for (int sl = 0; sl < SW; ++sl) {
       const float is[2] = {ist[0] * inv[sl], ist[1] * inv[sl]};
       m2[sl] = tail_epilogue(sub_tile<1>(y, sl), is, bt);
     }
-    __syncthreads();
-    if (lane < 4 * SW) mx[(s0 + (lane >> 2)) * MX_SLOTS + np + 2 * (lane & 3)] = (lane >> 2) ? m2[1] : m2[0];
+    wave_max_n(m2);
+    __syncthreads();
+    if (lane < 4 * SW) mx[(s0 + (lane >> 2)) * MX_SLOTS + np + 2 * (lane & 3)] = (lane >> 2) ? m2[SW - 1] : m2[0];
     float* xb = lds + s0 * D2::XSS + (2 + 4 * g) * D2::XSTR + c0;
 #pragma unroll
     for (int sl = 0; sl < SW; ++sl)
@@ -1404,12 +1485,16 @@
     rd_taps<G64, 1, 1, 2, true, false, NS, RDC>(xe, res, va64, wt0, wt0, ring);
     rd_ring_load<G64, 1, RDC>(ring, wt1p);
     rd_taps<G64, 1, 2, 2, true, false, NS, RDC>(xo, res, va64, wt1p, wt1p, ring);
+    float m[NS];
 #pragma unroll
     for (int sm = 0; sm < NS; ++sm) {
       const float s0[1] = {is0 * inv[sm]}, s1[1] = {is1 * inv[sm]};
-      const float m = tail_up_epilogue(sub_tile<1>(xe, sm), sub_tile<1>(xo, sm), s0, s1, bt);
-      if (lane == 0) mx[sm * MX_SLOTS + wave] = m;
-    }
+      m[sm] = tail_up_epilogue(sub_tile<1>(xe, sm), sub_tile<1>(xo, sm), s0, s1, bt);
+    }
+    wave_max_n(m);
+#pragma unroll
+    for (int sm = 0; sm < NS; ++sm)
+      if (lane == 0) mx[sm * MX_SLOTS + wave] = m[sm];
   }
 }
 
@@ -1615,7 +1700,7 @@
     rd_taps<GB, 2, 1, 2, true, false, 2, 2>(e, res, vaB, wt0, wt0, ring2);
     rd_ring_load<GB, 2, 2>(ring2, wt1);
     rd_taps<GB, 2, 2, 2, true, false, 2, 2>(o, res, vaB, wt1, wt1, ring2);
-    const DynScale df = dyn_scale(tail_up_epilogue(e, o, is0, is1, bt));
+    const DynScale df = dyn_scale(wave_max(tail_up_epilogue(e, o, is0, is1, bt)));
     inv_f = df.inv;
     wave_lds_fence();
     rw_zero_halo<GF>(slab, 64, lane, true);
@@ -1755,7 +1840,7 @@
     rd_taps<GB, 2, 1, 2, true, false, 1, 2>(e, res, vaB, wt0, wt0, ring2);
     rd_ring_load<GB, 2, 2>(ring2, wt1);
     rd_taps<GB, 2, 2, 2, true, false, 1, 2>(o, res, vaB, wt1, wt1, ring2);
-    const float m = tail_up_epilogue(e, o, is0, is1, bt);
+    const float m = wave_max(tail_up_epilogue(e, o, is0, is1, bt));
     const DynScale df = dyn_scale(half_sample_max(mx, sp, hf, lane, m));
     inv_f = df.inv;
     rw_zero_halo<GF>(slab, 64, lane, hf == 0);
```

Result: no change. 97850, median of 2 (+0.0%).
